# miczi/OpticalFlowHS

Hardware: AMD Instinct MI355X
Metric: Mpixel*iterations/sec (Horn-Schunck: derivative pass + Jacobi u/v sweeps, frames resident in HBM) (higher is better)
Workload: dtype f32; 1 GPU; a stream of 1920x1080 translating-texture pairs resident in HBM, a new pair every step (two seed pairs alternating), lambda 1, 100 Jacobi iterations, ITER|EPS (eps 1e-6) termination; width=1920, height=1080, iters=100, pairs_per_gpu=1, kernel=strip, fuse_steps=20, threads=1024, rows_per_lane_or_groups=5, tiles_per_launch=243, lds_bytes=131328, hipgraph=True, termination=ITER|EPS (eps 1e-6), loop=stream, call=hsflow_pipeline_submit_device, 6 slots on 2 streams, eps_rerun=0

## Files before the change

include/hsflow.h:

```cpp
#ifndef HSFLOW_H_
#define HSFLOW_H_

#include <stddef.h>
#include <stdint.h>

#ifdef __cplusplus
extern "C" {
#endif

#define HSFLOW_VERSION_MAJOR 0
#define HSFLOW_VERSION_MINOR 7

#define HSFLOW_OK 0
#define HSFLOW_E_ARG 1
#define HSFLOW_E_SIZE 2
#define HSFLOW_E_DEVICE 3
#define HSFLOW_E_OOM 4
#define HSFLOW_E_STATE 5
#define HSFLOW_E_NOTERM 6

#define HSFLOW_TERM_ITER 1
#define HSFLOW_TERM_EPS 2

#define HSFLOW_MODE_CV 0
// ... 7 lines not shown
#define HSFLOW_KERNEL_STRIP 3
#define HSFLOW_KERNEL_FOLD 4
#define HSFLOW_KERNEL_PERSIST 5

typedef struct hsflow_ctx hsflow_ctx;

typedef struct hsflow_params {
    uint32_t struct_size;
    int32_t mode;
    float lambda;
    float alpha;
    int32_t term_type;
    int32_t max_iter;
    double epsilon;
    int32_t use_previous;
    int32_t kernel;
    int32_t fuse_steps;
    int32_t tile_w;
    int32_t tile_h;
    int32_t threads;
    int32_t strip_rows;
    int32_t reuse_derivatives;
    int32_t use_graph;
    int32_t profile;
} hsflow_params;

typedef struct hsflow_info {
    uint32_t struct_size;
    int32_t width, height, n_pairs, pitch;
    int32_t iterations_done;
    float last_eps;
    int32_t kernel;
    int32_t fuse_steps, tile_w, tile_h, threads, groups_per_thread;
    int32_t tiles;
    int32_t lds_bytes;
    int32_t jacobi_launches;
    float deriv_ms;
    float jacobi_ms;
    float solve_ms;
    int32_t eps_rerun;
    int32_t deriv_fused;
    int32_t persistent;
} hsflow_info;


void hsflow_default_params(hsflow_params *p);

int hsflow_create(hsflow_ctx **out, int device, int width, int height, int n_pairs, void *stream,
                  int own_stream);
int hsflow_destroy(hsflow_ctx *ctx);
int hsflow_set_row_origin(hsflow_ctx *ctx, int first_row);

int hsflow_set_cu_share(hsflow_ctx *ctx, int compute_units);

int hsflow_set_async_reduce(hsflow_ctx *ctx, int on);

int hsflow_wait_solve(hsflow_ctx *ctx);


int hsflow_set_eps_rows(hsflow_ctx *ctx, int first_row, int rows);
int hsflow_solve_probe(hsflow_ctx *ctx, const hsflow_params *params, float *sweep_eps);
int hsflow_take_verdict(hsflow_ctx *ctx, int *proven);


int hsflow_set_frames_u8(hsflow_ctx *ctx, int pair, const uint8_t *prev, size_t prev_stride,
                         const uint8_t *curr, size_t curr_stride);
int hsflow_set_frames_u8_async(hsflow_ctx *ctx, int pair, const uint8_t *prev, size_t prev_stride,
                               const uint8_t *curr, size_t curr_stride);
int hsflow_set_frames_u8_device(hsflow_ctx *ctx, int pair, const void *d_prev, size_t prev_stride,
                                const void *d_curr, size_t curr_stride);
int hsflow_set_frames_bgr8(hsflow_ctx *ctx, int pair, const uint8_t *prev_bgr, size_t prev_stride,
                           const uint8_t *curr_bgr, size_t curr_stride, int blur3x3);
int hsflow_set_frames_gray8_blur(hsflow_ctx *ctx, int pair, const uint8_t *prev, size_t prev_stride,
                                 const uint8_t *curr, size_t curr_stride);
int hsflow_set_frames_bgr8_async(hsflow_ctx *ctx, int pair, const uint8_t *prev_bgr, size_t prev_stride,
                                 const uint8_t *curr_bgr, size_t curr_stride, int blur3x3);
int hsflow_set_frames_gray8_blur_async(hsflow_ctx *ctx, int pair, const uint8_t *prev, size_t prev_stride,
                                       const uint8_t *curr, size_t curr_stride);
int hsflow_push_frame_u8(hsflow_ctx *ctx, int pair, const uint8_t *next, size_t next_stride);


int hsflow_solve(hsflow_ctx *ctx, const hsflow_params *params);
int hsflow_solve_async(hsflow_ctx *ctx, const hsflow_params *params);
int hsflow_synchronize(hsflow_ctx *ctx);


int hsflow_get_flow(hsflow_ctx *ctx, int pair, float *u, size_t u_stride, float *v, size_t v_stride);
int hsflow_get_flow_async(hsflow_ctx *ctx, int pair, float *u, size_t u_stride, float *v, size_t v_stride);
int hsflow_flow_view_device(hsflow_ctx *ctx, int pair, const float **d_u, const float **d_v, size_t *stride_bytes);
int hsflow_get_flow_device(hsflow_ctx *ctx, int pair, int row0, int nrows, void *d_u,
                           size_t u_stride, void *d_v, size_t v_stride);
int hsflow_set_flow_device(hsflow_ctx *ctx, int pair, int row0, int nrows, const void *d_u,
                           size_t u_stride, const void *d_v, size_t v_stride);
int hsflow_get_derivatives(hsflow_ctx *ctx, int pair, float *dx, float *dy, float *dt,
                           size_t stride);
int hsflow_get_frames_u8(hsflow_ctx *ctx, int pair, uint8_t *prev, size_t prev_stride,
                         uint8_t *curr, size_t curr_stride);


#define HSFLOW_RENDER_CV 0
#define HSFLOW_RENDER_CL 1
typedef struct hsflow_render_params {
    uint32_t struct_size;
    int32_t step;
    float threshold, scale;
    uint8_t dot_rgb[3], line_rgb[3], pad[2];
} hsflow_render_params;
void hsflow_default_render_params(hsflow_render_params *rp, int preset);
int hsflow_render_flow_device(hsflow_ctx *ctx, int pair, const hsflow_render_params *rp, void *d_rgb, size_t stride);
int hsflow_render_flow(hsflow_ctx *ctx, int pair, const hsflow_render_params *rp, uint8_t *rgb, size_t stride);
int hsflow_render_line_pixels(int x0, int y0, int x1, int y1, int width, int height, int32_t *xy, int capacity);


#define HSFLOW_VERIFY_TINY 1e-30f
typedef struct hsflow_plane_diff {
    uint64_t differing, failing, nonfinite;
    int64_t first_failing;
    float max_abs_diff;
    uint32_t max_ulp;
} hsflow_plane_diff;

int hsflow_compare_planes_host(const float *a, size_t a_stride, const float *b, size_t b_stride, int width, int height,
                               hsflow_plane_diff *out);

int hsflow_compare_flow_device(hsflow_ctx *ctx, int pair, const void *d_u, size_t u_stride, const void *d_v, size_t v_stride,
                               hsflow_plane_diff *u, hsflow_plane_diff *v);

typedef struct hsflow_verify_report {
    uint32_t struct_size;
    int32_t ok;
    int32_t pair;
    int32_t iterations_done;
    int32_t iterations_ref;
    int32_t reserved;
    hsflow_plane_diff u, v;
    uint64_t deriv_differing;
    int64_t deriv_first;
} hsflow_verify_report;

int hsflow_verify(hsflow_ctx *ctx, int pair, hsflow_verify_report *report);


int hsflow_get_info(hsflow_ctx *ctx, hsflow_info *info);
int hsflow_get_info_ex(hsflow_ctx *ctx, hsflow_info *info, int measure_last_eps);
const char *hsflow_last_error(hsflow_ctx *ctx);
const char *hsflow_status_string(int status);
int hsflow_version(void);
int hsflow_device_count(int *count);


int hsflow_host_alloc(void **out, size_t bytes);
int hsflow_host_free(void *p);
int hsflow_host_register(void *p, size_t bytes);
int hsflow_host_unregister(void *p);


typedef struct hsflow_pipeline hsflow_pipeline;
int hsflow_pipeline_create(hsflow_pipeline **out, int device, int width, int height, int depth);
int hsflow_pipeline_create_lanes(hsflow_pipeline **out, int device, int width, int height, int depth, int lanes);
int hsflow_pipeline_destroy(hsflow_pipeline *pl);
int hsflow_pipeline_submit(hsflow_pipeline *pl, const uint8_t *prev, size_t prev_stride,
                           const uint8_t *curr, size_t curr_stride, float *u, size_t u_stride,
                           float *v, size_t v_stride, const hsflow_params *params, uint64_t *ticket);
#define HSFLOW_FRAMES_GRAY8 0
#define HSFLOW_FRAMES_GRAY8_BLUR 1
#define HSFLOW_FRAMES_BGR8 2
#define HSFLOW_FRAMES_BGR8_BLUR 3
int hsflow_pipeline_submit_ex(hsflow_pipeline *pl, int format, const uint8_t *prev, size_t prev_stride,
                              const uint8_t *curr, size_t curr_stride, float *u, size_t u_stride,
                              float *v, size_t v_stride, const hsflow_params *params, uint64_t *ticket);
int hsflow_pipeline_submit_device(hsflow_pipeline *pl, const void *d_prev, size_t prev_stride, const void *d_curr,
                                  size_t curr_stride, const hsflow_params *params, uint64_t *ticket);
int hsflow_pipeline_flow_device(hsflow_pipeline *pl, uint64_t ticket, const float **d_u, const float **d_v, size_t *stride_bytes);
int hsflow_pipeline_wait(hsflow_pipeline *pl, uint64_t ticket);
int hsflow_pipeline_render(hsflow_pipeline *pl, uint64_t ticket, const hsflow_render_params *rp, uint8_t *rgb, size_t stride);
int hsflow_pipeline_render_device(hsflow_pipeline *pl, uint64_t ticket, const hsflow_render_params *rp, void *d_rgb, size_t stride);
int hsflow_pipeline_verify(hsflow_pipeline *pl, uint64_t ticket, hsflow_verify_report *report);
int hsflow_pipeline_info(hsflow_pipeline *pl, uint64_t ticket, hsflow_info *info);
int hsflow_pipeline_drain(hsflow_pipeline *pl);
int hsflow_pipeline_depth(hsflow_pipeline *pl);
const char *hsflow_pipeline_last_error(hsflow_pipeline *pl);


typedef struct hsflow_multi hsflow_multi;
int hsflow_multi_create(hsflow_multi **out, const int *devices, int ndev, int width, int height, int depth);
int hsflow_multi_destroy(hsflow_multi *m);
int hsflow_multi_devices(hsflow_multi *m);
int hsflow_multi_submit(hsflow_multi *m, int format, const uint8_t *prev, size_t prev_stride, const uint8_t *curr, size_t curr_stride,
                        float *u, size_t u_stride, float *v, size_t v_stride, const hsflow_params *params, uint64_t *ticket);
int hsflow_multi_wait(hsflow_multi *m, uint64_t ticket);
int hsflow_multi_drain(hsflow_multi *m);
const char *hsflow_multi_last_error(hsflow_multi *m);

typedef struct hsflow_slab hsflow_slab;
int hsflow_slab_create(hsflow_slab **out, const int *devices, int nslab, int width, int height, int halo);
int hsflow_slab_destroy(hsflow_slab *s);
int hsflow_slab_count(hsflow_slab *s);
int hsflow_slab_rows(hsflow_slab *s, int k, int *lo, int *hi);
int hsflow_slab_set_frames_u8(hsflow_slab *s, const uint8_t *prev, size_t prev_stride, const uint8_t *curr, size_t curr_stride);
int hsflow_slab_solve(hsflow_slab *s, const hsflow_params *params);
int hsflow_slab_exchanges(hsflow_slab *s);
int hsflow_slab_iterations_done(hsflow_slab *s);
int hsflow_slab_eps_measured(hsflow_slab *s);
int hsflow_slab_create_overlapped(hsflow_slab **out, const int *devices, int ndev, int width, int height, int halo);
int hsflow_slab_get_flow(hsflow_slab *s, float *u, size_t u_stride, float *v, size_t v_stride);
const char *hsflow_slab_last_error(hsflow_slab *s);

int hsflow_plan_query(int width, int height, int n_pairs, const hsflow_params *params, hsflow_info *info);


int hsflow_calc_optical_flow_hs_8u32f(const uint8_t *prev, const uint8_t *curr, int img_step,
                                      int width, int height, int use_previous, float *velx,
                                      float *vely, int vel_step, float lambda, int term_type,
                                      int max_iter, double epsilon);

void hsflow_release_cached(void);

#ifdef __cplusplus
}
#endif
#endif
```

opticalflowhs_amd/_lib.py:

```python
import ctypes
import os

HERE = os.path.dirname(os.path.abspath(__file__))
LIB_PATH = os.environ.get("HSFLOW_LIB_PATH") or os.path.join(HERE, "libhsflow.so")

OK, E_ARG, E_SIZE, E_DEVICE, E_OOM, E_STATE, E_NOTERM = range(7)
TERM_ITER, TERM_EPS = 1, 2
MODE_CV, MODE_CLASSIC, MODE_CLASSIC_AS_SHIPPED = 0, 1, 2
KERNEL_AUTO, KERNEL_SIMPLE, KERNEL_FUSED, KERNEL_STRIP, KERNEL_FOLD, KERNEL_PERSIST = 0, 1, 2, 3, 4, 5
FRAMES_GRAY8, FRAMES_GRAY8_BLUR, FRAMES_BGR8, FRAMES_BGR8_BLUR = 0, 1, 2, 3
RENDER_CV, RENDER_CL = 0, 1


class HsflowParams(ctypes.Structure):
    _fields_ = [("struct_size", ctypes.c_uint32), ("mode", ctypes.c_int32),
                ("lambda_", ctypes.c_float), ("alpha", ctypes.c_float),
                ("term_type", ctypes.c_int32), ("max_iter", ctypes.c_int32),
                ("epsilon", ctypes.c_double), ("use_previous", ctypes.c_int32),
                ("kernel", ctypes.c_int32), ("fuse_steps", ctypes.c_int32),
                ("tile_w", ctypes.c_int32), ("tile_h", ctypes.c_int32),
                ("threads", ctypes.c_int32), ("strip_rows", ctypes.c_int32),
                ("reuse_derivatives", ctypes.c_int32), ("use_graph", ctypes.c_int32),
                ("profile", ctypes.c_int32)]


class HsflowInfo(ctypes.Structure):
    _fields_ = [("struct_size", ctypes.c_uint32), ("width", ctypes.c_int32),
                ("height", ctypes.c_int32), ("n_pairs", ctypes.c_int32), ("pitch", ctypes.c_int32),
                ("iterations_done", ctypes.c_int32), ("last_eps", ctypes.c_float),
                ("kernel", ctypes.c_int32), ("fuse_steps", ctypes.c_int32),
                ("tile_w", ctypes.c_int32), ("tile_h", ctypes.c_int32), ("threads", ctypes.c_int32),
                ("groups_per_thread", ctypes.c_int32), ("tiles", ctypes.c_int32),
                ("lds_bytes", ctypes.c_int32), ("jacobi_launches", ctypes.c_int32),
                ("deriv_ms", ctypes.c_float), ("jacobi_ms", ctypes.c_float),
                ("solve_ms", ctypes.c_float), ("eps_rerun", ctypes.c_int32),
                ("deriv_fused", ctypes.c_int32), ("persistent", ctypes.c_int32)]


class HsflowRenderParams(ctypes.Structure):
    _fields_ = [("struct_size", ctypes.c_uint32), ("step", ctypes.c_int32),
                ("threshold", ctypes.c_float), ("scale", ctypes.c_float),
                ("dot_rgb", ctypes.c_uint8 * 3), ("line_rgb", ctypes.c_uint8 * 3), ("pad", ctypes.c_uint8 * 2)]


class HsflowPlaneDiff(ctypes.Structure):
    _fields_ = [("differing", ctypes.c_uint64), ("failing", ctypes.c_uint64), ("nonfinite", ctypes.c_uint64),
                ("first_failing", ctypes.c_int64), ("max_abs_diff", ctypes.c_float), ("max_ulp", ctypes.c_uint32)]

    def as_dict(self):
        return {name: getattr(self, name) for name, _ in self._fields_}


class HsflowVerifyReport(ctypes.Structure):
    _fields_ = [("struct_size", ctypes.c_uint32), ("ok", ctypes.c_int32), ("pair", ctypes.c_int32),
                ("iterations_done", ctypes.c_int32), ("iterations_ref", ctypes.c_int32), ("reserved", ctypes.c_int32),
                ("u", HsflowPlaneDiff), ("v", HsflowPlaneDiff),
                ("deriv_differing", ctypes.c_uint64), ("deriv_first", ctypes.c_int64)]


VERIFY_TINY = 1e-30

_vp, _i, _sz = ctypes.c_void_p, ctypes.c_int, ctypes.c_size_t
_pp = ctypes.POINTER(HsflowParams)
_rp = ctypes.POINTER(HsflowRenderParams)
_dp = ctypes.POINTER(HsflowPlaneDiff)
_vr = ctypes.POINTER(HsflowVerifyReport)

PROTOTYPES = {
    "hsflow_default_params": (None, [_pp]),
    "hsflow_create": (_i, [ctypes.POINTER(_vp), _i, _i, _i, _i, _vp, _i]),
    "hsflow_destroy": (_i, [_vp]),
    "hsflow_set_row_origin": (_i, [_vp, _i]),
    "hsflow_set_cu_share": (_i, [_vp, _i]),
    "hsflow_set_async_reduce": (_i, [_vp, _i]),
    "hsflow_set_eps_rows": (_i, [_vp, _i, _i]),
    "hsflow_solve_probe": (_i, [_vp, _pp, ctypes.POINTER(ctypes.c_float)]),
    "hsflow_take_verdict": (_i, [_vp, ctypes.POINTER(_i)]),
    "hsflow_set_frames_u8": (_i, [_vp, _i, _vp, _sz, _vp, _sz]),
    "hsflow_set_frames_u8_async": (_i, [_vp, _i, _vp, _sz, _vp, _sz]),
    "hsflow_set_frames_u8_device": (_i, [_vp, _i, _vp, _sz, _vp, _sz]),
    "hsflow_set_frames_bgr8": (_i, [_vp, _i, _vp, _sz, _vp, _sz, _i]),
    "hsflow_set_frames_gray8_blur": (_i, [_vp, _i, _vp, _sz, _vp, _sz]),
    "hsflow_set_frames_bgr8_async": (_i, [_vp, _i, _vp, _sz, _vp, _sz, _i]),
    "hsflow_set_frames_gray8_blur_async": (_i, [_vp, _i, _vp, _sz, _vp, _sz]),
    "hsflow_push_frame_u8": (_i, [_vp, _i, _vp, _sz]),
    "hsflow_solve": (_i, [_vp, _pp]),
    "hsflow_solve_async": (_i, [_vp, _pp]),
    "hsflow_synchronize": (_i, [_vp]),
    "hsflow_wait_solve": (_i, [_vp]),
    "hsflow_get_flow": (_i, [_vp, _i, _vp, _sz, _vp, _sz]),
    "hsflow_get_flow_async": (_i, [_vp, _i, _vp, _sz, _vp, _sz]),
    "hsflow_flow_view_device": (_i, [_vp, _i, ctypes.POINTER(_vp), ctypes.POINTER(_vp), ctypes.POINTER(_sz)]),
    "hsflow_get_flow_device": (_i, [_vp, _i, _i, _i, _vp, _sz, _vp, _sz]),
    "hsflow_set_flow_device": (_i, [_vp, _i, _i, _i, _vp, _sz, _vp, _sz]),
    "hsflow_get_derivatives": (_i, [_vp, _i, _vp, _vp, _vp, _sz]),
    "hsflow_get_frames_u8": (_i, [_vp, _i, _vp, _sz, _vp, _sz]),
    "hsflow_default_render_params": (None, [_rp, _i]),
    "hsflow_render_flow_device": (_i, [_vp, _i, _rp, _vp, _sz]),
    "hsflow_render_flow": (_i, [_vp, _i, _rp, _vp, _sz]),
    "hsflow_render_line_pixels": (_i, [_i, _i, _i, _i, _i, _i, ctypes.POINTER(ctypes.c_int32), _i]),
    "hsflow_compare_planes_host": (_i, [_vp, _sz, _vp, _sz, _i, _i, _dp]),
    "hsflow_compare_flow_device": (_i, [_vp, _i, _vp, _sz, _vp, _sz, _dp, _dp]),
    "hsflow_verify": (_i, [_vp, _i, _vr]),
    "hsflow_pipeline_verify": (_i, [_vp, ctypes.c_uint64, _vr]),
    "hsflow_get_info": (_i, [_vp, ctypes.POINTER(HsflowInfo)]),
    "hsflow_get_info_ex": (_i, [_vp, ctypes.POINTER(HsflowInfo), _i]),
    "hsflow_last_error": (ctypes.c_char_p, [_vp]),
    "hsflow_status_string": (ctypes.c_char_p, [_i]),
    "hsflow_version": (_i, []),
    "hsflow_device_count": (_i, [ctypes.POINTER(_i)]),
    "hsflow_release_cached": (None, []),
    "hsflow_plan_query": (_i, [_i, _i, _i, _pp, ctypes.POINTER(HsflowInfo)]),
    "hsflow_host_alloc": (_i, [ctypes.POINTER(_vp), _sz]),
    "hsflow_host_free": (_i, [_vp]),
    "hsflow_host_register": (_i, [_vp, _sz]),
    "hsflow_host_unregister": (_i, [_vp]),
    "hsflow_pipeline_create": (_i, [ctypes.POINTER(_vp), _i, _i, _i, _i]),
    "hsflow_pipeline_create_lanes": (_i, [ctypes.POINTER(_vp), _i, _i, _i, _i, _i]),
    "hsflow_pipeline_destroy": (_i, [_vp]),
    "hsflow_pipeline_submit": (_i, [_vp, _vp, _sz, _vp, _sz, _vp, _sz, _vp, _sz, _pp, ctypes.POINTER(ctypes.c_uint64)]),
    "hsflow_pipeline_submit_ex": (_i, [_vp, _i, _vp, _sz, _vp, _sz, _vp, _sz, _vp, _sz, _pp, ctypes.POINTER(ctypes.c_uint64)]),
    "hsflow_pipeline_submit_device": (_i, [_vp, _vp, _sz, _vp, _sz, _pp, ctypes.POINTER(ctypes.c_uint64)]),
    "hsflow_pipeline_flow_device": (_i, [_vp, ctypes.c_uint64, ctypes.POINTER(_vp), ctypes.POINTER(_vp), ctypes.POINTER(_sz)]),
    "hsflow_pipeline_wait": (_i, [_vp, ctypes.c_uint64]),
    "hsflow_pipeline_render": (_i, [_vp, ctypes.c_uint64, _rp, _vp, _sz]),
    "hsflow_pipeline_render_device": (_i, [_vp, ctypes.c_uint64, _rp, _vp, _sz]),
    "hsflow_pipeline_info": (_i, [_vp, ctypes.c_uint64, ctypes.POINTER(HsflowInfo)]),
    "hsflow_pipeline_drain": (_i, [_vp]),
    "hsflow_pipeline_depth": (_i, [_vp]),
    "hsflow_pipeline_last_error": (ctypes.c_char_p, [_vp]),
    "hsflow_multi_create": (_i, [ctypes.POINTER(_vp), ctypes.POINTER(_i), _i, _i, _i, _i]),
    "hsflow_multi_destroy": (_i, [_vp]),
    "hsflow_multi_devices": (_i, [_vp]),
    "hsflow_multi_submit": (_i, [_vp, _i, _vp, _sz, _vp, _sz, _vp, _sz, _vp, _sz, _pp, ctypes.POINTER(ctypes.c_uint64)]),
    "hsflow_multi_wait": (_i, [_vp, ctypes.c_uint64]),
    "hsflow_multi_drain": (_i, [_vp]),
    "hsflow_multi_last_error": (ctypes.c_char_p, [_vp]),
    "hsflow_slab_create": (_i, [ctypes.POINTER(_vp), ctypes.POINTER(_i), _i, _i, _i, _i]),
    "hsflow_slab_destroy": (_i, [_vp]),
    "hsflow_slab_count": (_i, [_vp]),
    "hsflow_slab_rows": (_i, [_vp, _i, ctypes.POINTER(_i), ctypes.POINTER(_i)]),
    "hsflow_slab_set_frames_u8": (_i, [_vp, _vp, _sz, _vp, _sz]),
    "hsflow_slab_solve": (_i, [_vp, _pp]),
    "hsflow_slab_exchanges": (_i, [_vp]),
    "hsflow_slab_iterations_done": (_i, [_vp]),
    "hsflow_slab_eps_measured": (_i, [_vp]),
    "hsflow_slab_create_overlapped": (_i, [ctypes.POINTER(_vp), ctypes.POINTER(_i), _i, _i, _i, _i]),
    "hsflow_slab_get_flow": (_i, [_vp, _vp, _sz, _vp, _sz]),
    "hsflow_slab_last_error": (ctypes.c_char_p, [_vp]),
    "hsflow_calc_optical_flow_hs_8u32f": (_i, [_vp, _vp, _i, _i, _i, _i, _vp, _vp, _i,
                                               ctypes.c_float, _i, _i, ctypes.c_double]),
}

_lib = None


def load():
    global _lib
    if _lib is not None:
        return _lib
    try:
        import torch
    except ImportError:
        pass
    if not os.path.exists(LIB_PATH):
        raise ImportError(
            "opticalflowhs_amd: %s is missing -- build it with `python opticalflowhs_amd/build.py` "
            "(hipcc, gfx950). There is no CPU fallback." % LIB_PATH)
    try:
        lib = ctypes.CDLL(LIB_PATH)
    except OSError as e:
        raise ImportError("opticalflowhs_amd: cannot load %s: %s" % (LIB_PATH, e))
    for name, (res, args) in PROTOTYPES.items():
        try:
            fn = getattr(lib, name)
        except AttributeError:
            raise ImportError("opticalflowhs_amd: %s does not export %s" % (LIB_PATH, name))
        fn.restype = res
        fn.argtypes = args
    _lib = lib
    return lib


class HsflowError(RuntimeError):
    def __init__(self, status, message):
        RuntimeError.__init__(self, "hsflow status %d: %s" % (status, message))
        self.status = status
```

opticalflowhs_amd/csrc/hs_context.hip.h:

```cpp
#pragma once

namespace {

constexpr int kMaxFuse = 32;
constexpr int kLdsLimit = 160 * 1024;
constexpr int kNumCU = 256;

thread_local std::string g_create_error;

struct FusedPlan {
    hsk::FusedGeom g;
    int NT, K, lds_bytes, tiles;
};

struct StripPlan {
    hsk::StripGeom g;
    int R, lds_bytes, tiles;
    int fold;
};

struct JPlan {
    int kind = 0;
    int T = 0;
    FusedPlan f{};
// ... 29 lines not shown
};

struct SolveSetup {
    float coeff;
    int kernel;
    bool multi;
    bool use_iter, use_eps;
    long long budget;
    int T;
    JPlan plan;
    bool persist;
    hsflow_params eff;
};

struct PlanKey {
    hsflow_params p;
    int async, exact;
};
struct PlanEntry {
    PlanKey key;
    SolveSetup S;
    hsflow_info info;
};

}

struct hsflow_ctx {
    int device = 0;
    int W = 0, H = 0, N = 0, P = 0;
    int org = 0;
    long long plane = 0;
    hipStream_t stream = nullptr;
    bool own_stream = false;
    uint8_t *dA = nullptr, *dB = nullptr;
    uint32_t *dCoef = nullptr;
    float *dE[3] = {nullptr, nullptr, nullptr};
    bool dE_valid = false;
    int coef_mode = -1;
    float *dU[2] = {nullptr, nullptr}, *dV[2] = {nullptr, nullptr};
    unsigned long long *dStamps = nullptr;
    unsigned *dEps = nullptr;
    unsigned *epsPtr = nullptr;
    float epsThr = 0.f;
    unsigned *hEps = nullptr;
    unsigned *hEpsDev = nullptr;
    size_t hEpsCap = 0;
    int epsStride = 1;
    unsigned *dEpsTiles = nullptr;
    size_t epsTilesCap = 0;
    float *dUb = nullptr, *dVb = nullptr;
    float *dUp = nullptr, *dVp = nullptr;
    unsigned *dFlags = nullptr;
    unsigned *hErr = nullptr, *hErrDev = nullptr;
    int persist_tiles = 0;
    bool persist_off = false;
    bool persist_unchecked = false;
    bool counted = false;
    int eps_row0 = 0, eps_rows = 0;
    std::vector<float> sweep_eps;
    unsigned *dSeq = nullptr, *hMark = nullptr, *hMarkDev = nullptr;
    float *dZero = nullptr;
    unsigned mark_issued = 0;
    bool last_marked = false;
    bool flow_after_mark = false;
    bool async_reduce = false;
    int cu_share = 0;
    int num_cu = 0;
    int max_grid_z = 65535;
    void *dScratch = nullptr;
    unsigned *dPrio = nullptr;
    bool prio_dirty = false;
    uint8_t *dRgb = nullptr;
    hipEvent_t evRender = nullptr;
    hsflow_params vparams;
    int vstate = 0;
    int v_org = 0, v_eps_row0 = 0, v_eps_rows = 0;
    hsflow_ctx *shadow = nullptr;
    bool borrowed = false;
    unsigned long long *dCmp = nullptr, *hCmp = nullptr;
    int cmp_cap = 0;
    hipEvent_t evVerify = nullptr;
    size_t scratch_bytes = 0;
    int cur = 0;
    bool frames_set = false;
    bool coef_valid = false;
    hsflow_info info;
    std::string err;
    struct Pending {
        bool active = false;
        hsflow_params params;
        int iters = 0, launches = 0, cur0 = 0;
        EpsLayout words;
        bool reduced = false;
        unsigned mark = 0;
        bool marked_by_reduce = false;
    } pend;
    struct LastLaunch {
        bool valid = false;
        JPlan plan;
        int zero_in = 0;
        float coeff = 0.f, eps_thr = 0.f;
        bool from_third = false;
    } lastl;
    bool force_exact = false;
    bool configuring = false;
    std::map<GraphKey, GraphEntry> graphs;
    std::vector<PlanEntry> plan_cache;
    std::vector<hipEvent_t> events;
};

namespace {

std::atomic<int> g_live_ctx[64];
constexpr int kMaxPersistTiles = 4096;

hsflow_ctx *g_oneshot = nullptr;
std::mutex g_oneshot_mutex;

int fail(hsflow_ctx *c, int code, const std::string &msg)
{
    if (c) c->err = msg; else g_create_error = msg;
    return code;
}

#define HS_HIP(c, call)                                                                           \
    do {                                                                                          \
        hipError_t e_ = (call);                                                                   \
        if (e_ != hipSuccess)                                                                     \
            return fail((c), e_ == hipErrorOutOfMemory ? HSFLOW_E_OOM : HSFLOW_E_DEVICE,          \
                        std::string(#call) + ": " + hipGetErrorString(e_));                       \
    } while (0)

int round_up(int v, int m) { return (v + m - 1) / m * m; }

}
```

opticalflowhs_amd/csrc/hs_kernels_strip.hip.h:

```cpp
#pragma once
#include <type_traits>

#ifndef HS_SCALED
#define HS_SCALED 1
#endif
#ifndef HS_UNROLL2_FOLD
#define HS_UNROLL2_FOLD 1
#endif
#ifndef HS_PEEL_LAST_STRIP
#define HS_PEEL_LAST_STRIP 1
#endif
#ifndef HS_PEEL_LAST_FOLD
#define HS_PEEL_LAST_FOLD 1
#endif
#ifndef HS_CORE_PRIO
#define HS_CORE_PRIO 1
#endif
#ifndef HS_SWEEP_STAMPS
#define HS_SWEEP_STAMPS 0
#endif
#ifndef HS_DIAG
#define HS_DIAG 0
#endif

// ... 47 lines not shown
}
__device__ __forceinline__ f4 load_f4_sc1(__amdgpu_buffer_rsrc_t rs, unsigned row_bytes, unsigned lane_bytes)
{
    return __builtin_bit_cast(f4, __builtin_amdgcn_raw_buffer_load_b128(rs, (int)lane_bytes, (int)row_bytes, 16));
}
__device__ __forceinline__ unsigned load_u32_sc1(const unsigned *p)
{
    return __hip_atomic_load(p, __ATOMIC_RELAXED, __HIP_MEMORY_SCOPE_AGENT);
}

__device__ __forceinline__ int hs_lane_now()
{
    unsigned m = ~0u;
    asm volatile("" : "+s"(m));
    return (int)__builtin_amdgcn_mbcnt_hi(m, __builtin_amdgcn_mbcnt_lo(m, 0u));
}

__device__ __forceinline__ f2 f2_fma(f2 a, f2 b, f2 c) { return __builtin_elementwise_fma(a, b, c); }
__device__ __forceinline__ f2 f2_swap(f2 a) { return __builtin_shufflevector(a, a, 1, 0); }
#if HS_SCALED
#define HS_DIFF(o, n) f2_fma((o), f2{4.0f, 4.0f}, -(n))
#define HS_DIFF1(o, n) fmaf(4.0f, (o), -(n))
#else
#define HS_DIFF(o, n) ((o) - (n))
#define HS_DIFF1(o, n) ((o) - (n))
#endif

struct RowCoef { f2 alP, alQ, beP, beQ, gaP, gaQ; };

struct Cross { f2 uP, uQ, vP, vQ; };

__device__ __forceinline__ f2 pk_add_swapped(f2 a, f2 b)
{
    f2 r;
    asm("v_pk_add_f32 %0, %1, %2 op_sel:[0,1] op_sel_hi:[1,0]" : "=v"(r) : "v"(a), "v"(b));
    return r;
}

template <int E>
__device__ __forceinline__ void cross_rows(Cross &s, const f2 cuP, const f2 cuQ, const f2 cvP, const f2 cvQ,
                                           const f2 duP, const f2 duQ, const f2 dvP, const f2 dvQ)
{
    if (E == 0) {
        s.uP = duP + cuQ; s.uQ = duQ + cuP;
        s.vP = dvP + cvQ; s.vQ = dvQ + cvP;
    } else {
        s.uQ = pk_add_swapped(duQ, cuQ);
        s.uP.x = duP.x + wave_from_prev_lane(cuP.y); s.uP.y = duP.y + wave_from_next_lane(cuP.x);
        s.vQ = pk_add_swapped(dvQ, cvQ);
        s.vP.x = dvP.x + wave_from_prev_lane(cvP.y); s.vP.y = dvP.y + wave_from_next_lane(cvP.x);
    }
}

template <int E>
__device__ __forceinline__ void strip_row_update(f2 &uP, f2 &uQ, f2 &vP, f2 &vQ, const Cross &sc, const Cross &sp, RowCoef &c)
{
    f2 tP, tQ, sP, sQ;
    if (E == 0) {
        tQ = pk_add_swapped(sc.uQ, sp.uQ);
        tP.x = sc.uP.x + wave_from_prev_lane(sp.uP.y); tP.y = sc.uP.y + wave_from_next_lane(sp.uP.x);
        sQ = pk_add_swapped(sc.vQ, sp.vQ);
        sP.x = sc.vP.x + wave_from_prev_lane(sp.vP.y); sP.y = sc.vP.y + wave_from_next_lane(sp.vP.x);
    } else {
        tP = sc.uP + sp.uQ; tQ = sc.uQ + sp.uP;
        sP = sc.vP + sp.vQ; sQ = sc.vQ + sp.vP;
    }
#if HS_SCALED
    const f2 ubP = tP, ubQ = tQ, vbP = sP, vbQ = sQ;
#else
    const f2 ubP = tP * 0.25f, ubQ = tQ * 0.25f, vbP = sP * 0.25f, vbQ = sQ * 0.25f;
#endif
    const f2 qP = f2_fma(c.alP, ubP, f2_fma(c.beP, vbP, c.gaP));
    const f2 qQ = f2_fma(c.alQ, ubQ, f2_fma(c.beQ, vbQ, c.gaQ));
    uP = f2_fma(-c.alP, qP, ubP);
    vP = f2_fma(-c.beP, qP, vbP);
    uQ = f2_fma(-c.alQ, qQ, ubQ);
    vQ = f2_fma(-c.beQ, qQ, vbQ);
#if HS_SCALED
    c.gaP *= 4.0f;
    c.gaQ *= 4.0f;
#endif
}

template <int R>
__device__ __forceinline__ void strip_derive(const uint8_t *__restrict__ fA, const uint8_t *__restrict__ fB,
                                             const StripGeom &g, long long base, int x0, int y0, int dir, bool xin,
                                             uint4 (&lc)[R])
{
    const int mode = xin ? 0 : ((x0 < 0 || (g.W & 3) == 0) ? 1 : 2);
    int xg = x0, xb[4] = {0, 0, 0, 0};
    unsigned flipx = 0;
    if (mode == 1) {
        xg = x0 < 0 ? -x0 - 4 : 2 * g.W - x0 - 4;
        if (xg < 0 || xg + 4 > g.W) xg = 0;
        flipx = 0xFu;
    } else if (mode == 2) {
#pragma unroll
        for (int k = 0; k < 4; k++) {
            xb[k] = mirror_index(x0 + k, g.W);
            if (x0 + k >= g.W) flipx |= 1u << k;
        }
    }
    uint32_t wa[R + 2], wbv[R];
#pragma unroll
    for (int j = 0; j < R + 2; j++)
        wa[j] = *(const uint32_t *)(fA + base + (long long)mirror_index(y0 + dir * (j - 1), g.H) * g.P + (mode == 2 ? 0 : xg));
#pragma unroll
    for (int r = 0; r < R; r++)
        wbv[r] = *(const uint32_t *)(fB + base + (long long)mirror_index(y0 + dir * r, g.H) * g.P + (mode == 2 ? 0 : xg));
    if (mode == 1) {
#pragma unroll
        for (int j = 0; j < R + 2; j++) wa[j] = __builtin_bswap32(wa[j]);
#pragma unroll
        for (int r = 0; r < R; r++) wbv[r] = __builtin_bswap32(wbv[r]);
    }
    if (__builtin_amdgcn_ballot_w64(mode == 2) != 0) {
        if (mode == 2) {
            auto bytes = [&](const uint8_t *row) -> uint32_t {
                return (uint32_t)row[xb[0]] | ((uint32_t)row[xb[1]] << 8) | ((uint32_t)row[xb[2]] << 16) | ((uint32_t)row[xb[3]] << 24);
            };
#pragma unroll
            for (int j = 0; j < R + 2; j++) wa[j] = bytes(fA + base + (long long)mirror_index(y0 + dir * (j - 1), g.H) * g.P);
#pragma unroll
            for (int r = 0; r < R; r++) wbv[r] = bytes(fB + base + (long long)mirror_index(y0 + dir * r, g.H) * g.P);
        }
    }
    int a[R + 2][6];
#pragma unroll
    for (int j = 0; j < R + 2; j++) {
        const uint32_t wd = wa[j];
        a[j][0] = (int)((uint32_t)__builtin_amdgcn_update_dpp(0, (int)wd, 0x138, 0xF, 0xF, true) >> 24);
        a[j][5] = (int)((uint32_t)__builtin_amdgcn_update_dpp(0, (int)wd, 0x130, 0xF, 0xF, true) & 0xFFu);
#pragma unroll
        for (int k = 0; k < 4; k++) a[j][k + 1] = (int)((wd >> (8 * k)) & 0xFFu);
    }
#pragma unroll
    for (int r = 0; r < R; r++) {
        const int y = y0 + dir * r;
        const uint32_t wb = wbv[r];
        const bool yflip = (y < 0 || y >= g.H) != (dir < 0);
        uint32_t o[4];
#pragma unroll
        for (int k = 0; k < 4; k++) {
            int ix8 = (a[r][k + 2] + 2 * a[r + 1][k + 2] + a[r + 2][k + 2]) - (a[r][k] + 2 * a[r + 1][k] + a[r + 2][k]);
            int iy8 = (a[r + 2][k] + 2 * a[r + 2][k + 1] + a[r + 2][k + 2]) - (a[r][k] + 2 * a[r][k + 1] + a[r][k + 2]);
            if ((flipx >> k) & 1u) ix8 = -ix8;
            if (yflip) iy8 = -iy8;
            o[k] = pack_deriv(ix8, iy8, (int)((wb >> (8 * k)) & 0xFFu) - a[r + 1][k + 1]);
        }
        lc[r] = make_uint4(o[0], o[1], o[2], o[3]);
    }
}

template <int R, int NTMAX, int EPS, int E0, bool DERIV, bool PERSIST = false>
__device__ __forceinline__ void strip_body(const uint32_t *__restrict__ coef,
                                                        const float *__restrict__ u_in,
                                                        const float *__restrict__ v_in,
                                                        float *__restrict__ u_out,
                                                        float *__restrict__ v_out, const StripGeom g,
                                                        const float ilambda,
                                                        unsigned *__restrict__ eps_out, const int eps_stride,
                                                        unsigned long long *__restrict__ stamps,
                                                        const float eps_thr, const uint8_t *__restrict__ fA,
                                                        const uint8_t *__restrict__ fB, uint32_t *__restrict__ coef_w,
                                                        const PersistArgs pa = PersistArgs())
{
    static_assert(!PERSIST || EPS == 0 || EPS == 2, "the persistent form runs plain or witness phases");
    extern __shared__ __attribute__((aligned(16))) float4 ex[];
    unsigned long long st0 = 0, sr0 = 0, st1 = 0, st2 = 0;
    if (stamps) { st0 = __builtin_amdgcn_s_memtime(); sr0 = __builtin_amdgcn_s_memrealtime(); }
    const int lane = threadIdx.x & 63;
    const int w = __builtin_amdgcn_readfirstlane(threadIdx.x >> 6);
    const int NW = g.NW;
    float *eps_lds = (float *)(ex + (size_t)2 * NW * 4 * 64);
    const int tpp = g.tiles_x * g.tiles_y;
    const int tile = xcd_contiguous_tile(blockIdx.x, gridDim.x);
    const int pair = tile / tpp;
    const int t2 = tile - pair * tpp;
    const int by = t2 / g.tiles_x, bx = t2 - by * g.tiles_x;
    const int x0 = bx * g.CW - g.HX + 4 * lane;
    const int y0 = by * g.CH - g.T + w * R;
    const long long base = (long long)pair * g.plane;
    const bool xin = (x0 >= 0) && (x0 + 3 < g.W);
    const bool rev = (R & 1) != 0 && ((y0 + g.org) & 1) != 0;
    auto img_row = [&](int r) { return rev ? R - 1 - r : r; };

    f2 uP[R], uQ[R], vP[R], vQ[R];
    RowCoef cf[R];
    float4 lu[R], lv[R];
    uint4 lc[R];
    const int rx0 = bx * g.CW - g.HX;
    const bool xedge = !(rx0 >= 0 && rx0 + 256 <= g.W);
    int xg = x0;
    bool xrev = false, slow = false;
    if (xedge && !xin) {
        if (x0 < 0 && -x0 <= g.W) { xg = -x0 - 4; xrev = true; }
        else if (x0 >= g.W && (g.W & 3) == 0 && 2 * g.W - x0 - 4 >= 0) { xg = 2 * g.W - x0 - 4; xrev = true; }
        else { xg = 0; slow = true; }
    }
#pragma unroll
    for (int r = 0; r < R; r++) {
        const long long off = base + (long long)mirror_index(y0 + img_row(r), g.H) * g.P + xg;
        const long long off_uv = g.zero_in ? (long long)xg : off;
        lc[r] = make_uint4(0u, 0u, 0u, 0u);
        if constexpr (!DERIV) {
            lu[r] = *(const float4 *)(u_in + off_uv);
            lv[r] = *(const float4 *)(v_in + off_uv);
            lc[r] = *(const uint4 *)(coef + off);
        } else {
            lu[r] = lv[r] = make_float4(0.f, 0.f, 0.f, 0.f);
        }
    }
    if constexpr (DERIV) {
        if (!g.zero_in) {
#pragma unroll
            for (int r = 0; r < R; r++) {
                const long long off = base + (long long)mirror_index(y0 + img_row(r), g.H) * g.P + xg;
                lu[r] = *(const float4 *)(u_in + off);
                lv[r] = *(const float4 *)(v_in + off);
            }
        }
    }
    auto unpack_row = [&](const int r) __attribute__((always_inline)) {
        const float4 lu_ = lu[r], lv_ = lv[r];
        const uint4 cw = lc[r];
        constexpr int iPx = 0, iPy = 3, iQx = 1, iQy = 2;
        const float lu4[4] = {lu_.x, lu_.y, lu_.z, lu_.w}, lv4[4] = {lv_.x, lv_.y, lv_.z, lv_.w};
        uP[r] = f2{lu4[iPx], lu4[iPy]}; uQ[r] = f2{lu4[iQx], lu4[iQy]};
        vP[r] = f2{lv4[iPx], lv4[iPy]}; vQ[r] = f2{lv4[iQx], lv4[iQy]};
        float al[4], be[4], ga[4];
        const uint32_t cc[4] = {cw.x, cw.y, cw.z, cw.w};
#pragma unroll
        for (int p = 0; p < 4; p++) sweep_coefs(cc[p], ilambda, al[p], be[p], ga[p]);
        cf[r].alP = f2{al[iPx], al[iPy]}; cf[r].alQ = f2{al[iQx], al[iQy]};
        cf[r].beP = f2{be[iPx], be[iPy]}; cf[r].beQ = f2{be[iQx], be[iQy]};
        cf[r].gaP = f2{ga[iPx], ga[iPy]} * (HS_SCALED ? 4.0f : 1.0f); cf[r].gaQ = f2{ga[iQx], ga[iQy]} * (HS_SCALED ? 4.0f : 1.0f);
    };
    if constexpr (!DERIV) {
#pragma unroll
        for (int r = 0; r < R; r++) unpack_row(r);
    }
    if (xedge) {
#pragma unroll
        for (int r = 0; r < R; r++) {
            if constexpr (DERIV) {
                if (xrev) {
                    lu[r] = make_float4(lu[r].w, lu[r].z, lu[r].y, lu[r].x);
                    lv[r] = make_float4(lv[r].w, lv[r].z, lv[r].y, lv[r].x);
                }
            } else {
                uP[r] = xrev ? f2_swap(uP[r]) : uP[r]; uQ[r] = xrev ? f2_swap(uQ[r]) : uQ[r];
                vP[r] = xrev ? f2_swap(vP[r]) : vP[r]; vQ[r] = xrev ? f2_swap(vQ[r]) : vQ[r];
                cf[r].alP = xrev ? f2_swap(cf[r].alP) : cf[r].alP; cf[r].alQ = xrev ? f2_swap(cf[r].alQ) : cf[r].alQ;
                cf[r].beP = xrev ? f2_swap(cf[r].beP) : cf[r].beP; cf[r].beQ = xrev ? f2_swap(cf[r].beQ) : cf[r].beQ;
                cf[r].gaP = xrev ? f2_swap(cf[r].gaP) : cf[r].gaP; cf[r].gaQ = xrev ? f2_swap(cf[r].gaQ) : cf[r].gaQ;
            }
        }
        if (__builtin_amdgcn_ballot_w64(slow) != 0) {
            if (slow) {
                const int xa = mirror_index(x0, g.W), xb = mirror_index(x0 + 1, g.W),
                          xc = mirror_index(x0 + 2, g.W), xd = mirror_index(x0 + 3, g.W);
#pragma unroll
                for (int r = 0; r < R; r++) {
                    const long long row = base + (long long)mirror_index(y0 + img_row(r), g.H) * g.P;
                    {
                        const float *uv = u_in + (g.zero_in ? 0 : row), *vv = v_in + (g.zero_in ? 0 : row);
                        lu[r] = make_float4(uv[xa], uv[xb], uv[xc], uv[xd]);
                        lv[r] = make_float4(vv[xa], vv[xb], vv[xc], vv[xd]);
                    }
                    if constexpr (!DERIV) {
                        const uint32_t *cv = coef + row;
                        lc[r] = make_uint4(cv[xa], cv[xb], cv[xc], cv[xd]);
                        unpack_row(r);
                    }
                }
            }
        }
    }
    if constexpr (DERIV) {
        strip_derive<R>(fA, fB, g, base, x0, rev ? y0 + R - 1 : y0, rev ? -1 : 1, xin, lc);
#pragma unroll
        for (int r = 0; r < R; r++) unpack_row(r);
    }
    unsigned rowcore = 0;
    int rdist[R];
#pragma unroll
    for (int r = 0; r < R; r++) {
        const int j = w * R + img_row(r), y = y0 + img_row(r);
        if (j >= g.T && j < g.T + g.CH && y >= 0 && y < g.H) rowcore |= 1u << r;
        rdist[r] = j < g.T ? g.T - j : (j >= g.T + g.CH ? j - (g.T + g.CH - 1) : 0);
    }
    const bool lanecore = (x0 >= 0) && (x0 < g.W) && (4 * lane >= g.HX) && (4 * lane < g.HX + g.CW);
    const int pr = g.W - 1 - x0;
    const int lane_kept = lane;
    constexpr bool LANE_HW = EPS != 0 || PERSIST;
#define lane (LANE_HW ? hs_lane_now() : lane_kept)
    unsigned epscore = 0;
    if (EPS != 0) {
#pragma unroll
        for (int r = 0; r < R; r++) {
            const int y = y0 + img_row(r);
            if (((rowcore >> r) & 1u) && y >= g.ey0 && y < g.ey1) epscore |= 1u << r;
        }
    }
    if (DERIV && lanecore) {
#pragma unroll
        for (int r = 0; r < R; r++)
            if ((rowcore >> r) & 1u) *(uint4 *)(coef_w + base + (long long)(y0 + img_row(r)) * g.P + x0) = lc[r];
    }

#define HS_ACT(r) (rdist[r] <= last)
#define HS_ROW(r, PE, SC, SP)                                                                      \
    do {                                                                                           \
        if (HS_ACT(r)) {                                                                           \
            f2 ouP, ouQ, ovP, ovQ;                                                                 \
            if (EM == 1) { ouP = uP[r]; ouQ = uQ[r]; ovP = vP[r]; ovQ = vQ[r]; }                   \
            if (HS_DIAG & 8) uP[r] += SC.uP + SP.uP;                                               \
            else strip_row_update<PE>(uP[r], uQ[r], vP[r], vQ[r], SC, SP, cf[r]);                  \
            if (EM == 1) {                                                                         \
                if ((epscore >> (r)) & 1u) {  \
                    const f2 dUP = HS_DIFF(ouP, uP[r]), dUQ = HS_DIFF(ouQ, uQ[r]), dVP = HS_DIFF(ovP, vP[r]), dVQ = HS_DIFF(ovQ, vQ[r]); \
                    if (!xedge) {  \
                        e = fmaxf(fmaxf(e, fabsf(dUP.x)), fabsf(dUP.y));                           \
                        e = fmaxf(fmaxf(e, fabsf(dUQ.x)), fabsf(dUQ.y));                           \
                        e = fmaxf(fmaxf(e, fabsf(dVP.x)), fabsf(dVP.y));                           \
                        e = fmaxf(fmaxf(e, fabsf(dVQ.x)), fabsf(dVQ.y));                           \
                    } else {                                                                       \
                         \
                        e = fmaxf(e, fmaxf(fabsf(dUP.x), fabsf(dVP.x)));                           \
                        if (pr >= 1) e = fmaxf(e, fmaxf(fabsf(dUQ.x), fabsf(dVQ.x)));              \
                        if (pr >= 2) e = fmaxf(e, fmaxf(fabsf(dUQ.y), fabsf(dVQ.y)));              \
                        if (pr >= 3) e = fmaxf(e, fmaxf(fabsf(dUP.y), fabsf(dVP.y)));              \
                    }                                                                              \
                }                                                                                  \
            }                                                                                      \
        }                                                                                          \
    } while (0)
#define HS_CROSS(S, PE, A, B)                                                                      \
    do {                                                                                           \
        if (HS_ACT(A) || HS_ACT(B)) {                                                              \
            if (HS_DIAG & 8) S.uP = uP[A] + uP[B];                                                 \
            else cross_rows<PE>(S, uP[A], uQ[A], vP[A], vQ[A], uP[B], uQ[B], vP[B], vQ[B]);        \
        }                                                                                          \
    } while (0)
#define HS_PUBLISH(buf)                                                                            \
    do {                                                                                           \
        float4 *exw = ex + ((size_t)((buf) * NW + w) * 4) * 64 + HS_LANE;                          \
        exw[0] = make_float4(uP[0].x, uP[0].y, uQ[0].x, uQ[0].y);                                  \
        exw[64] = make_float4(vP[0].x, vP[0].y, vQ[0].x, vQ[0].y);                                 \
        exw[128] = make_float4(uP[R - 1].x, uP[R - 1].y, uQ[R - 1].x, uQ[R - 1].y);                \
        exw[192] = make_float4(vP[R - 1].x, vP[R - 1].y, vQ[R - 1].x, vQ[R - 1].y);                \
    } while (0)

    if (stamps) st1 = __builtin_amdgcn_s_memtime();
    const bool nrev = (R & 1) != 0 && !rev;
    const int wa = w > 0 ? w - 1 : w, sa = w > 0 ? (nrev ? 0 : 2) : 0;
    const int wb = w < NW - 1 ? w + 1 : w, sb = w < NW - 1 ? (nrev ? 2 : 0) : 2;
    const int wu = rev ? wb : wa, su = rev ? sb : sa;
    const int wd = rev ? wa : wb, sd = rev ? sa : sb;
    int seen_n = 0;
    const unsigned long long wit_mask = (epscore & 1u) ? __builtin_amdgcn_ballot_w64(lanecore) : 0ull;
    const int core_here = min(g.CH, g.H - by * g.CH);
    const int wit_lo = (g.T + R - 1) / R, wit_n = (g.T + core_here) / R - wit_lo;
// ... 213 lines not shown
                if (nx >= 0 && nx < g.tiles_x && ny >= 0 && ny < g.tiles_y) nb = pair * tpp + ny * g.tiles_x + nx;
            } else if (lane == 8) nb = (int)gridDim.x;
            const unsigned long long t0 = __builtin_amdgcn_s_memrealtime();
            int dead = 0;
            for (;;) {
                unsigned v = target;
                if (nb >= 0) v = load_u32_sc1(pa.flags + nb);
                const bool aborted = lane == 8 && v != 0u;
                const bool behind = lane < 8 && (int)(v - target) < 0;
                if (__builtin_amdgcn_ballot_w64(aborted) != 0) { dead = 1; break; }
                if (__builtin_amdgcn_ballot_w64(behind) == 0) break;
                if (__builtin_amdgcn_s_memrealtime() - t0 > (unsigned long long)pa.wait_ticks) {
                    dead = 1;
                    if (lane == 0) {
                        __hip_atomic_store(pa.flags + gridDim.x, 1u, __ATOMIC_RELAXED, __HIP_MEMORY_SCOPE_AGENT);
                        __hip_atomic_store(pa.err, 1u, __ATOMIC_RELAXED, __HIP_MEMORY_SCOPE_SYSTEM);
                    }
                    break;
                }
                __builtin_amdgcn_s_sleep(4);
            }
            if (lane == 0) *dead_lds = dead;
        }
        __syncthreads();
        if (__builtin_amdgcn_readfirstlane(*dead_lds)) return;
        if (stamps) { const unsigned long long t = __builtin_amdgcn_s_memtime(); pt_wait += t - pt0; pt0 = t; }
        {
            f4 tu[R], tv[R];
#pragma unroll
            for (int r = 0; r < R; r++) {
                const unsigned row = 4u * (unsigned)(base + (long long)mirror_index(y0 + img_row(r), g.H) * g.P);
                tu[r] = f4{uP[r].x, uQ[r].x, uQ[r].y, uP[r].y};
                tv[r] = f4{vP[r].x, vQ[r].x, vQ[r].y, vP[r].y};
                if (!((rowcore >> r) & 1u) || !lanecore) {
                    tu[r] = load_f4_sc1(pu, row, 4u * (unsigned)xgx);
                    tv[r] = load_f4_sc1(pv, row, 4u * (unsigned)xgx);
                }
            }
#pragma unroll
            for (int r = 0; r < R; r++) {
                if (xrevx) {
                    tu[r] = f4{tu[r].w, tu[r].z, tu[r].y, tu[r].x};
                    tv[r] = f4{tv[r].w, tv[r].z, tv[r].y, tv[r].x};
                }
                uP[r] = f2{tu[r].x, tu[r].w}; uQ[r] = f2{tu[r].y, tu[r].z};
                vP[r] = f2{tv[r].x, tv[r].w}; vQ[r] = f2{tv[r].y, tv[r].z};
            }
        }
        ph++;
    }
    }
#undef HS_ROW
#undef HS_ACT
#undef HS_CROSS
#undef HS_PUBLISH
#undef HS_LANE
#undef lane
    if (stamps && threadIdx.x == 0) {
        __builtin_amdgcn_s_waitcnt(0);
        unsigned long long *o = stamps + (size_t)blockIdx.x * 8;
        o[0] = st0; o[1] = st1; o[2] = st2; o[3] = __builtin_amdgcn_s_memtime();
        o[4] = sr0; o[5] = __builtin_amdgcn_s_memrealtime();
        o[6] = (unsigned long long)__builtin_amdgcn_s_getreg(((4 - 1) << 11) | (0 << 6) | 20);
        o[7] = (unsigned long long)tile;
        if (PERSIST && gridDim.x <= 8192) {
            unsigned long long *q = stamps + (size_t)gridDim.x * 8 + (size_t)blockIdx.x * 32;
            q[0] = pt_sweep; q[1] = pt_pub; q[2] = pt_wait; q[3] = pt_load; q[4] = pt_first - st1; q[5] = o[3] - st2;
        }
    }
}

template <int R, int NTMAX, int EPS, int E0>
__global__ __launch_bounds__(NTMAX) void k_jacobi_strip(const uint32_t *__restrict__ coef,
                                                        const float *__restrict__ u_in,
                                                        const float *__restrict__ v_in,
                                                        float *__restrict__ u_out,
                                                        float *__restrict__ v_out, const StripGeom g,
                                                        const float ilambda,
                                                        unsigned *__restrict__ eps_out, const int eps_stride,
                                                        unsigned long long *__restrict__ stamps,
                                                        const float eps_thr)
{
    strip_body<R, NTMAX, EPS, E0, false>(coef, u_in, v_in, u_out, v_out, g, ilambda, eps_out, eps_stride, stamps, eps_thr,
                                     nullptr, nullptr, nullptr);
}

template <int R, int NTMAX, int EPS, int E0>
__global__ __launch_bounds__(NTMAX) void k_jacobi_strip_deriv(const uint8_t *__restrict__ fA,
                                                              const uint8_t *__restrict__ fB,
                                                              uint32_t *__restrict__ coef_w,
                                                              const float *__restrict__ u_in,
                                                              const float *__restrict__ v_in,
                                                              float *__restrict__ u_out,
                                                              float *__restrict__ v_out, const StripGeom g,
                                                              const float ilambda,
                                                              unsigned *__restrict__ eps_out, const int eps_stride,
                                                              unsigned long long *__restrict__ stamps,
                                                              const float eps_thr)
{
    strip_body<R, NTMAX, EPS, E0, true>(nullptr, u_in, v_in, u_out, v_out, g, ilambda, eps_out, eps_stride, stamps, eps_thr,
                                    fA, fB, coef_w);
}

template <int R, int NTMAX, int EPS, int E0, bool DERIV>
__global__ __launch_bounds__(NTMAX) void k_jacobi_strip_persist(const uint8_t *__restrict__ fA,
                                                                const uint8_t *__restrict__ fB,
                                                                uint32_t *coef_rw,
                                                                const float *__restrict__ u_in,
                                                                const float *__restrict__ v_in, const StripGeom g,
                                                                const float ilambda,
                                                                unsigned *__restrict__ eps_out, const int eps_stride,
                                                                unsigned long long *__restrict__ stamps,
                                                                const float eps_thr, const PersistArgs pa)
{
    strip_body<R, NTMAX, EPS, E0, DERIV, true>(coef_rw, u_in, v_in, nullptr, nullptr, g, ilambda, eps_out, eps_stride, stamps, eps_thr,
                                               fA, fB, coef_rw, pa);
}

__device__ __forceinline__ float lane_xor32(float x, bool lower)
{
    const unsigned b = __float_as_uint(x);
    const auto r = __builtin_amdgcn_permlane32_swap(b, b, false, false);
    return __uint_as_float(lower ? r[0] : r[1]);
}

template <int R, int NTMAX, int EPS, int E0, bool DERIV>
__device__ __forceinline__ void fold_body(const uint32_t *__restrict__ coef,
                                                       const float *__restrict__ u_in,
                                                       const float *__restrict__ v_in,
                                                       float *__restrict__ u_out,
                                                       float *__restrict__ v_out, const StripGeom g,
                                                       const float ilambda,
                                                       unsigned *__restrict__ eps_out, const int eps_stride,
                                                       unsigned long long *__restrict__ stamps,
                                                       const float eps_thr, const uint8_t *__restrict__ fA,
                                                       const uint8_t *__restrict__ fB, uint32_t *__restrict__ coef_w)
{
    extern __shared__ __attribute__((aligned(16))) float4 ex[];
    unsigned long long st0 = 0, sr0 = 0, st1 = 0, st2 = 0;
    if (stamps) { st0 = __builtin_amdgcn_s_memtime(); sr0 = __builtin_amdgcn_s_memrealtime(); }
    const int lane = threadIdx.x & 63, hl = lane & 31;
    const bool lower = lane >= 32;
    const int w = __builtin_amdgcn_readfirstlane(threadIdx.x >> 6);
    const int NW = g.NW;
    float *eps_lds = (float *)(ex + (size_t)2 * NW * 2 * 2 * 32);
    const int tpp = g.tiles_x * g.tiles_y;
    const int tile = xcd_contiguous_tile(blockIdx.x, gridDim.x);
    const int pair = tile / tpp;
    const int t2 = tile - pair * tpp;
    const int by = t2 / g.tiles_x, bx = t2 - by * g.tiles_x;
    const int rx0 = bx * g.CW - g.HX;
    const int x0 = rx0 + 4 * hl;
    const int yb = by * g.CH - g.T + w * 2 * R;
    const long long base = (long long)pair * g.plane;
    const bool xin = (x0 >= 0) && (x0 + 3 < g.W);

    f2 uP[R], uQ[R], vP[R], vQ[R];
    RowCoef cf[R];
    float4 lu[R], lv[R];
    uint4 lc[R];
    const bool side = !(rx0 >= 0 && rx0 + 128 <= g.W);
    int xg = x0;
    bool rev = false, slow = false;
    if (side && !xin) {
        if (x0 < 0 && -x0 <= g.W) { xg = -x0 - 4; rev = true; }
        else if (x0 >= g.W && (g.W & 3) == 0 && 2 * g.W - x0 - 4 >= 0) { xg = 2 * g.W - x0 - 4; rev = true; }
        else { xg = 0; slow = true; }
    }
#pragma unroll
    for (int r = 0; r < R; r++) {
        const int y = yb + (lower ? 2 * R - 1 - r : r);
        const long long off = base + (long long)mirror_index(y, g.H) * g.P + xg;
        const long long off_uv = g.zero_in ? (long long)xg : off;
        lc[r] = make_uint4(0u, 0u, 0u, 0u);
        if constexpr (!DERIV) {
            lu[r] = *(const float4 *)(u_in + off_uv);
            lv[r] = *(const float4 *)(v_in + off_uv);
            lc[r] = *(const uint4 *)(coef + off);
        } else {
            lu[r] = lv[r] = make_float4(0.f, 0.f, 0.f, 0.f);
        }
    }
    if constexpr (DERIV) {
        if (!g.zero_in) {
#pragma unroll
            for (int r = 0; r < R; r++) {
                const int y = yb + (lower ? 2 * R - 1 - r : r);
                const long long off = base + (long long)mirror_index(y, g.H) * g.P + xg;
                lu[r] = *(const float4 *)(u_in + off);
                lv[r] = *(const float4 *)(v_in + off);
            }
        }
    }
    auto unpack_row = [&](const int r) __attribute__((always_inline)) {
        constexpr int iPx = 0, iPy = 3, iQx = 1, iQy = 2;
        const float lu4[4] = {lu[r].x, lu[r].y, lu[r].z, lu[r].w}, lv4[4] = {lv[r].x, lv[r].y, lv[r].z, lv[r].w};
        uP[r] = f2{lu4[iPx], lu4[iPy]}; uQ[r] = f2{lu4[iQx], lu4[iQy]};
        vP[r] = f2{lv4[iPx], lv4[iPy]}; vQ[r] = f2{lv4[iQx], lv4[iQy]};
        float al[4], be[4], ga[4];
// ... 264 lines not shown
```

opticalflowhs_amd/csrc/hs_plan_launch.hip.h:

```cpp
#pragma once

namespace {
int eps_row0(const hsflow_ctx *c) { return c->eps_rows > 0 ? c->eps_row0 : 0; }
int eps_row1(const hsflow_ctx *c) { return c->eps_rows > 0 ? c->eps_row0 + c->eps_rows : c->H; }
bool eps_windowed(const hsflow_ctx *c) { return c->eps_rows > 0 && (c->eps_row0 > 0 || c->eps_rows < c->H); }

int plan_cus(const hsflow_ctx *c) { return c->cu_share > 0 ? c->cu_share : kNumCU; }
bool plan_shared(const hsflow_ctx *c) { return c->cu_share > 0 && c->cu_share < kNumCU; }

bool grid_fits(long long tiles, int threads) { return tiles * threads <= 0xFFFFFFFFLL; }

bool make_plan(const hsflow_ctx *c, int T, int tw, int th, int nt, FusedPlan &best)
{
    const int W = c->W, H = c->H;
    const int HX = round_up(T, 4);
    double best_cost = 1e300;
    bool found = false;
    const int nts[3] = {1024, 512, 256};
    for (int nti = 0; nti < 3; nti++) {
        const int NT = nts[nti];
        if (nt && nt != NT) continue;
        const int Kmax = NT == 1024 ? 3 : 4;
        const int wg_per_cu = 1;
        const int cw_lo = tw ? tw : 4, cw_hi = tw ? tw : std::min(round_up(W, 4), 1024);
// ... 234 lines not shown
    const double valu = std::max(wps, 1.0) * R * instr_per_row * cpi * (1.0 - 0.45 * halo_frac);
    const double exchange = 300.0 + (fold ? 12.0 : 20.0) * NW * conc;
    const double sweep = valu + exchange;
    double load = 2050.0 + 0.4 * 256.0 * R * NW * conc;
    if (conc > 1) load *= 0.4;
    const double r = (double)tiles / (double)slots;
    const double rounds = plan_shared(c) ? std::max(1.0, r) : conc == 1 ? std::ceil(r) : std::max(1.0, r + 0.7);
    return 6000.0 + 6e-4 * 8.0 * image_pixels + rounds * (load + T * sweep);
}

bool make_strip_plan(const hsflow_ctx *c, int T, int rows, int threads, int fold, StripPlan &best, double *cost_out = nullptr)
{
    const int W = c->W, H = c->H;
    const int HX = round_up(T, 4);
    const int CW = (fold ? 128 : 256) - 2 * HX;
    if (CW < 4) return false;
    double best_cost = 1e300;
    bool found = false;
    for (int R = 1; R <= 8; R++) {
        if (rows && rows != R) continue;
        for (int NW = 1; NW <= strip_max_waves(R, fold); NW++) {
            if (threads && threads != NW * 64) continue;
            const int CH = NW * R * (fold ? 2 : 1) - 2 * T;
            if (CH < 1) continue;
            const int lds = NW * (fold ? 4096 : 8192) + (fold ? 128 : 256);
            if (lds > kLdsLimit) continue;
            const int tx = (W + CW - 1) / CW, ty = (H + CH - 1) / CH;
            const long long tiles = (long long)tx * ty * c->N;
            if (!grid_fits(tiles, NW * 64)) continue;
            const double cost = strip_launch_cost(c, T, R, NW, tiles, fold, (double)W * H * c->N);
            if (cost < best_cost - 1e-9) {
                best_cost = cost;
                found = true;
                best.R = R;
                best.fold = fold;
                best.lds_bytes = lds;
                best.tiles = (int)tiles;
                hsk::StripGeom &g = best.g;
                g.W = W; g.H = H; g.P = c->P; g.plane = c->plane;
                g.T = T; g.HX = HX; g.CW = CW; g.CH = CH; g.NW = NW;
                g.tiles_x = tx; g.tiles_y = ty; g.zero_in = 0; g.org = c->org;
                g.ey0 = eps_row0(c); g.ey1 = eps_row1(c);
            }
        }
    }
    if (cost_out) *cost_out = best_cost;
    return found;
}

int pick_strip_T(const hsflow_ctx *c, int iters, const hsflow_params &p, int fold, double *total_out = nullptr)
{
    double best = 1e300;
    int bestT = 1;
    for (int T = 1; T <= std::min(iters, 24); T++) {
        StripPlan sp;
        double cfull = 0, ctail = 0;
        if (!make_strip_plan(c, T, p.strip_rows, p.threads, fold, sp, &cfull)) continue;
        const int rem = iters % T;
        if (rem && !make_strip_plan(c, rem, p.strip_rows, p.threads, fold, sp, &ctail)) continue;
        const double total = (iters / T) * cfull + (rem ? ctail : 0.0);
        if (total < best) { best = total; bestT = T; }
    }
    if (total_out) *total_out = best;
    return bestT;
}

int strip_phase(const StripPlan &p) { return (p.fold || (p.R & 1) == 0) ? ((p.g.T + p.g.org) & 1) : 0; }

template <int R, int NTMAX, int EPS, bool FOLD, bool DERIV, int E0>
constexpr auto strip_kernel()
{
    if constexpr (FOLD && DERIV) return hsk::k_jacobi_fold_deriv<R, NTMAX, EPS, E0>;
    else if constexpr (FOLD) return hsk::k_jacobi_fold<R, NTMAX, EPS, E0>;
    else if constexpr (DERIV) return hsk::k_jacobi_strip_deriv<R, NTMAX, EPS, E0>;
    else return hsk::k_jacobi_strip<R, NTMAX, EPS, E0>;
}

template <int R, int NTMAX, EpsMode EPS, bool FOLD, bool DERIV, int E0>
hipError_t launch_strip_k(const hsflow_ctx *c, const StripPlan &p, const float *ui, const float *vi, float *uo, float *vo, float coeff)
{
    constexpr auto kern = strip_kernel<R, NTMAX, (int)EPS, FOLD, DERIV, E0>();
    if (p.g.zero_in) ui = vi = c->dZero;
    unsigned long long *stamps = p.tiles <= 65536 ? c->dStamps : nullptr;
    if constexpr (DERIV)
        return launch_lds<kern>(c, p.tiles, p.g.NW * 64, p.lds_bytes, c->dA, c->dB, c->dCoef, ui, vi, uo, vo, p.g, coeff, c->epsPtr,
                                c->epsStride, stamps, c->epsThr);
    else
        return launch_lds<kern>(c, p.tiles, p.g.NW * 64, p.lds_bytes, c->dCoef, ui, vi, uo, vo, p.g, coeff, c->epsPtr, c->epsStride,
                                stamps, c->epsThr);
}

template <int R, int NTMAX, EpsMode EPS, bool FOLD, bool DERIV>
hipError_t launch_strip_t(const hsflow_ctx *c, const StripPlan &p, const float *ui, const float *vi, float *uo, float *vo, float coeff)
{
    if constexpr (FOLD || (R & 1) == 0) {
        if (strip_phase(p)) return launch_strip_k<R, NTMAX, EPS, FOLD, DERIV, 1>(c, p, ui, vi, uo, vo, coeff);
    }
    return launch_strip_k<R, NTMAX, EPS, FOLD, DERIV, 0>(c, p, ui, vi, uo, vo, coeff);
}

constexpr int strip_ntmax(int R, bool fold, bool narrow)
{
    return R <= 4 ? 1024 : R == 5 ? (fold || narrow ? 768 : 1024) : R == 6 ? (fold ? 512 : 768) : 512;
}

template <int R, EpsMode EPS, bool FOLD, bool DERIV>
hipError_t launch_strip_r(const hsflow_ctx *c, const StripPlan &p, const float *ui, const float *vi, float *uo, float *vo, float coeff)
{
    constexpr int NT = strip_ntmax(R, FOLD, false), NT_NARROW = strip_ntmax(R, FOLD, EPS != EpsMode::None);
    if constexpr (NT_NARROW != NT) {
        if (p.g.NW <= 12) return launch_strip_t<R, NT_NARROW, EPS, FOLD, DERIV>(c, p, ui, vi, uo, vo, coeff);
    }
    return launch_strip_t<R, NT, EPS, FOLD, DERIV>(c, p, ui, vi, uo, vo, coeff);
}

template <EpsMode EPS, bool FOLD, bool DERIV>
hipError_t launch_strip_e(const hsflow_ctx *c, const StripPlan &p, const float *ui, const float *vi, float *uo, float *vo, float coeff)
{
#ifdef HS_DIAG_MIN
    if constexpr (!FOLD && !DERIV && EPS == EpsMode::None) {
        if (p.R == 4) return launch_strip_r<4, EPS, FOLD, DERIV>(c, p, ui, vi, uo, vo, coeff);
        if (p.R == 5) return launch_strip_r<5, EPS, FOLD, DERIV>(c, p, ui, vi, uo, vo, coeff);
        if (p.R == 6) return launch_strip_r<6, EPS, FOLD, DERIV>(c, p, ui, vi, uo, vo, coeff);
    }
#else
    switch (p.R) {
    case 1: return launch_strip_r<1, EPS, FOLD, DERIV>(c, p, ui, vi, uo, vo, coeff);
    case 2: return launch_strip_r<2, EPS, FOLD, DERIV>(c, p, ui, vi, uo, vo, coeff);
    case 3: return launch_strip_r<3, EPS, FOLD, DERIV>(c, p, ui, vi, uo, vo, coeff);
    case 4: return launch_strip_r<4, EPS, FOLD, DERIV>(c, p, ui, vi, uo, vo, coeff);
    case 5: return launch_strip_r<5, EPS, FOLD, DERIV>(c, p, ui, vi, uo, vo, coeff);
    case 6: return launch_strip_r<6, EPS, FOLD, DERIV>(c, p, ui, vi, uo, vo, coeff);
    }
    if constexpr (!DERIV) {
        if (p.R == 7) return launch_strip_r<7, EPS, FOLD, DERIV>(c, p, ui, vi, uo, vo, coeff);
        if (p.R == 8) return launch_strip_r<8, EPS, FOLD, DERIV>(c, p, ui, vi, uo, vo, coeff);
    }
#endif
    return hipErrorInvalidConfiguration;
}

template <EpsMode EPS>
hipError_t launch_strip_m(const hsflow_ctx *c, const StripPlan &p, bool deriv, const float *ui, const float *vi, float *uo, float *vo,
                          float coeff)
{
    if constexpr (EPS != EpsMode::EverySweep) {
        if (deriv) return p.fold ? launch_strip_e<EPS, true, true>(c, p, ui, vi, uo, vo, coeff)
                                 : launch_strip_e<EPS, false, true>(c, p, ui, vi, uo, vo, coeff);
    }
    if (deriv) return hipErrorInvalidConfiguration;
    return p.fold ? launch_strip_e<EPS, true, false>(c, p, ui, vi, uo, vo, coeff)
                  : launch_strip_e<EPS, false, false>(c, p, ui, vi, uo, vo, coeff);
}

constexpr unsigned kPersistWaitTicks = 5000000u;

const char *persist_obstacle(const hsflow_ctx *c, const StripPlan &sp, int iters, const hsflow_params &p, bool async, bool use_eps)
{
    static const bool off = getenv("HSFLOW_NO_PERSIST") != nullptr;
    const hsk::StripGeom &g = sp.g;
    if (off) return "HSFLOW_NO_PERSIST is set";
    if (c->persist_off) return "a persistent launch timed out on this context earlier";
    if (sp.fold) return "the folded kernel has no persistent form";
    if (sp.R != 5 || g.NW * 64 > 1024) return "the persistent form is compiled for 5 rows per lane";
    if (iters <= g.T) return "a single phase";
    if ((g.W & 3) != 0 || g.W < 256 || g.H < g.NW * sp.R) return "the frame must be at least one region large and its width a multiple of 4";
    if (g.CH < g.T || g.CW < g.HX) return "the halo reaches past the neighbouring tiles";
// ... 170 lines not shown
```

opticalflowhs_amd/csrc/hs_runtime.hip.h:

```cpp
#pragma once

namespace {
constexpr size_t kMaxGraphs = 32;
void drop_graphs(hsflow_ctx *c)
{
    if (c->graphs.empty()) return;
    hipStreamSynchronize(c->stream);
    for (auto &kv : c->graphs) {
        if (kv.second.exec) hipGraphExecDestroy(kv.second.exec);
        if (kv.second.graph) hipGraphDestroy(kv.second.graph);
    }
    c->graphs.clear();
}

void trim_graph_cache(hsflow_ctx *c)
{
    if (c->graphs.size() >= kMaxGraphs) drop_graphs(c);
}

int check_ctx(hsflow_ctx *c, int pair)
{
    if (!c) return fail(nullptr, HSFLOW_E_ARG, "null context");
    if (pair < 0 || pair >= c->N) return fail(c, HSFLOW_E_ARG, "pair index out of range");
    if (hipSetDevice(c->device) != hipSuccess) return fail(c, HSFLOW_E_DEVICE, "hipSetDevice failed");
    (void)hipGetLastError();
    return HSFLOW_OK;
}

struct Profiler {
    hsflow_ctx *c;
    bool on;
    std::vector<std::pair<int, size_t>> marks;
    size_t used = 0;
    hipEvent_t ev(size_t i)
    {
        while (c->events.size() <= i) {
            hipEvent_t e;
            if (hipEventCreate(&e) != hipSuccess) return nullptr;
            c->events.push_back(e);
        }
        return c->events[i];
    }
    void begin(int kind)
    {
        if (!on) return;
        marks.push_back({kind, used});
        hipEventRecord(ev(used), c->stream);
        used++;
    }
    void end()
    {
        if (!on) return;
        hipEventRecord(ev(used), c->stream);
        used++;
    }
    void collect()
    {
        if (!on || marks.empty()) return;
        hipStreamSynchronize(c->stream);
        float d = 0, j = 0, t = 0;
        for (auto &m : marks) {
            float ms = 0;
            hipEventElapsedTime(&ms, c->events[m.second], c->events[m.second + 1]);
            (m.first == 0 ? d : j) += ms;
        }
        hipEventElapsedTime(&t, c->events[marks.front().second], c->events[used - 1]);
        c->info.deriv_ms = d;
        c->info.jacobi_ms = j;
        c->info.solve_ms = t;
    }
};

int persist_reserve(hsflow_ctx *c)
{
    const size_t px = (size_t)c->plane * c->N;
    if (!c->dUp) HS_HIP(c, hipMalloc((void **)&c->dUp, px * sizeof(float)));
    if (!c->dVp) HS_HIP(c, hipMalloc((void **)&c->dVp, px * sizeof(float)));
    if (!c->dFlags) {
        HS_HIP(c, hipMalloc((void **)&c->dFlags, (size_t)(kMaxPersistTiles + 1) * sizeof(unsigned)));
        c->persist_tiles = 0;
    }
    if (!c->hErr) {
        HS_HIP(c, hipHostMalloc((void **)&c->hErr, 64, hipHostMallocMapped | hipHostMallocCoherent));
        HS_HIP(c, hipHostGetDevicePointer((void **)&c->hErrDev, c->hErr, 0));
        *c->hErr = 0u;
    }
    return HSFLOW_OK;
}

int persist_prepare_flags(hsflow_ctx *c, int tiles)
{
    if (c->persist_tiles == tiles) return HSFLOW_OK;
    HS_HIP(c, hipMemsetAsync(c->dFlags, 0, (size_t)(kMaxPersistTiles + 1) * sizeof(unsigned), c->stream));
    c->persist_tiles = tiles;
    return HSFLOW_OK;
}

void persist_failed(hsflow_ctx *c)
{
    if (c->hErr) *c->hErr = 0u;
    c->persist_tiles = 0;
    c->persist_off = true;
    c->persist_unchecked = false;
    c->coef_valid = false;
    c->plan_cache.clear();
}

bool persist_error(const hsflow_ctx *c) { return c->hErr && *(volatile unsigned *)c->hErr != 0u; }

bool persist_gave_up(hsflow_ctx *c)
{
    const bool gave_up = c->persist_unchecked && persist_error(c);
    c->persist_unchecked = false;
    if (gave_up) persist_failed(c);
    return gave_up;
}

int enqueue_persist(hsflow_ctx *c, const StripPlan &sp0, int iters, EpsMode eps, bool deriv, int zero_in, float coeff)
{
    StripPlan sp = sp0;
    sp.g.zero_in = zero_in;
    hsk::PersistArgs pa;
    const int T = sp.g.T;
    pa.n_phase = (iters + T - 1) / T;
    pa.T_last = iters - (pa.n_phase - 1) * T;
    pa.flags = c->dFlags;
    pa.err = c->hErrDev;
    static const char *ticks_env = getenv("HSFLOW_PERSIST_WAIT_TICKS");
    pa.wait_ticks = ticks_env ? (unsigned)strtoul(ticks_env, nullptr, 10) : kPersistWaitTicks;
    const int a = c->cur, b = a ^ 1;
    const int lastb = (pa.n_phase - 1) & 1;
    pa.ub[lastb] = c->dU[b]; pa.vb[lastb] = c->dV[b];
    pa.ub[lastb ^ 1] = c->dUp; pa.vb[lastb ^ 1] = c->dVp;
    HS_HIP(c, launch_persist(c, sp, pa, eps, deriv, c->dU[a], c->dV[a], coeff));
    c->cur = b;
    return HSFLOW_OK;
}

int configure_persist(hsflow_ctx *c, const StripPlan &sp, EpsMode eps, bool deriv, float coeff)
{
    c->configuring = true;
    const hipError_t e = launch_persist(c, sp, hsk::PersistArgs{}, eps, deriv, nullptr, nullptr, coeff);
    c->configuring = false;
    HS_HIP(c, e);
    return HSFLOW_OK;
}

int enqueue_fixed(hsflow_ctx *c, const hsflow_params &p, float coeff, int iters, int kernel, int T,
                  const JPlan *plan, const JPlan *tail_plan, Profiler &prof, bool do_deriv, bool zero_flow, bool persist = false)
{
    int zero_in = zero_flow ? 1 : 0;
    if (zero_flow) c->cur = 0;
    bool fuse = do_deriv && !p.profile && kernel != HSFLOW_KERNEL_SIMPLE &&
                strip_deriv_fusable(c, iters >= T ? *plan : *tail_plan);
    if (do_deriv && !fuse) {
        prof.begin(0);
        HS_HIP(c, launch_deriv(c));
        prof.end();
    }
    int left = iters, launches = 0;
    if (persist) {
        prof.begin(1);
        const int st = enqueue_persist(c, plan->s, iters, EpsMode::None, fuse, zero_in, coeff);
        prof.end();
        if (st) return st;
        left = 0;
        launches = 1;
    }
    while (left > 0) {
        const int a = c->cur, b = a ^ 1;
        if (kernel == HSFLOW_KERNEL_SIMPLE) {
            prof.begin(1);
            HS_HIP(c, launch_simple(c, false, c->dU[a], c->dV[a], c->dU[b], c->dV[b], coeff, zero_in));
            prof.end();
            left -= 1;
        } else {
            const JPlan *pl = (left >= T) ? plan : tail_plan;
            prof.begin(1);
            HS_HIP(c, launch_j(c, *pl, EpsMode::None, c->dU[a], c->dV[a], c->dU[b], c->dV[b], coeff, zero_in, fuse));
            prof.end();
            fuse = false;
            left -= pl->T;
        }
        c->cur = b;
        zero_in = 0;
        launches++;
    }
    c->info.jacobi_launches = launches;
    return HSFLOW_OK;
}

int eps_reserve(hsflow_ctx *c, int sweeps, int stride)
{
    const size_t need = (size_t)sweeps * stride;
    if (c->epsTilesCap < need) {
        drop_graphs(c);
        hipFree(c->dEpsTiles);
        c->dEpsTiles = nullptr; c->epsTilesCap = 0;
        HS_HIP(c, hipMalloc((void **)&c->dEpsTiles, need * sizeof(unsigned)));
        c->epsTilesCap = need;
    }
    if (c->hEpsCap < (size_t)sweeps) {
        drop_graphs(c);
        HS_HIP(c, hipStreamSynchronize(c->stream));
        if (c->hEps) hipHostFree(c->hEps);
        c->hEps = c->hEpsDev = nullptr; c->hEpsCap = 0;
        const size_t cap = std::max<size_t>(256, (size_t)sweeps * 2);
        HS_HIP(c, hipHostMalloc((void **)&c->hEps, cap * sizeof(unsigned), hipHostMallocMapped | hipHostMallocCoherent));
        HS_HIP(c, hipHostGetDevicePointer((void **)&c->hEpsDev, c->hEps, 0));
        c->hEpsCap = cap;
    }
    c->epsStride = stride;
    return HSFLOW_OK;
}

int eps_clear(hsflow_ctx *c, int sweeps, int stride)
{
    HS_HIP(c, hipMemsetAsync(c->dEpsTiles, 0, (size_t)sweeps * stride * sizeof(unsigned), c->stream));
    return HSFLOW_OK;
}

int eps_prepare(hsflow_ctx *c, int sweeps, int stride)
{
    const int st = eps_reserve(c, sweeps, stride);
    return st ? st : eps_clear(c, sweeps, stride);
}

int eps_collect_enqueue(hsflow_ctx *c, const EpsLayout &w, bool mark = false)
{
    c->epsPtr = c->dEps;
    c->epsStride = 1;
    if (c->configuring) return HSFLOW_OK;
    hipLaunchKernelGGL(hsk::k_eps_reduce, dim3(w.slots), dim3(256), 0, c->stream, c->dEpsTiles, w.stride, c->hEpsDev, w.n_first,
                       w.cnt_first, w.cnt_last, mark ? c->dSeq : nullptr, mark ? c->hMarkDev : nullptr);
    HS_HIP(c, hipGetLastError());
    return HSFLOW_OK;
}

int eps_collect(hsflow_ctx *c, int sweeps, std::vector<unsigned> &host)
{
    int st = eps_collect_enqueue(c, EpsLayout{sweeps, c->epsStride, 0, 0, c->epsStride});
    if (st) return st;
    HS_HIP(c, hipStreamSynchronize(c->stream));
    host.assign(c->hEps, c->hEps + sweeps);
    return HSFLOW_OK;
}

bool witness_proven(const unsigned *w, int slots, double epsilon, float *last, bool last_is_exact)
{
    float e = 0.f;
    for (int i = 0; i < slots; i++) {
        std::memcpy(&e, &w[i], sizeof(float));
        if (!((double)e >= epsilon) && !(last_is_exact && i == slots - 1)) return false;
    }
    *last = e;
    return true;
}

int plan_eps_stride(int kernel, const JPlan &pl) { return (kernel == HSFLOW_KERNEL_STRIP || kernel == HSFLOW_KERNEL_FOLD) ? pl.s.tiles : 1; }

constexpr int kStampTiles = 65536;
void dump_stamps(hsflow_ctx *c, int tiles)
{
    const char *path = getenv("HSFLOW_DEBUG_STAMPS");
    if (!path || !c->dStamps) return;
    tiles = std::min(tiles, kStampTiles);
    std::vector<unsigned long long> h((size_t)tiles * 8);
    if (hipMemcpy(h.data(), c->dStamps, h.size() * 8, hipMemcpyDeviceToHost) != hipSuccess) return;
    FILE *f = fopen(path, "a");
// ... 39 lines not shown
```

opticalflowhs_amd/csrc/hs_solve.hip.h:

```cpp
#pragma once

namespace {
int solve_impl(hsflow_ctx *c, const hsflow_params *pp, bool async);

int check_persist(hsflow_ctx *c)
{
    if (!persist_gave_up(c)) return HSFLOW_OK;
    return fail(c, HSFLOW_E_DEVICE, "a persistent launch of an asynchronous solve timed out (another grid on the device?): its flow is invalid; "
                                    "this context now launches per fuse_steps iterations, solve again");
}

int wait_marker(hsflow_ctx *c, unsigned target)
{
    if (!c->hMark) { HS_HIP(c, hipStreamSynchronize(c->stream)); return HSFLOW_OK; }
    const auto t0 = std::chrono::steady_clock::now();
    unsigned spins = 0;
    while ((int)(__atomic_load_n(c->hMark, __ATOMIC_ACQUIRE) - target) < 0) {
        if ((++spins & 1023u) == 0 && std::chrono::steady_clock::now() - t0 > std::chrono::seconds(2)) {
            HS_HIP(c, hipStreamSynchronize(c->stream));
            break;
        }
    }
    return HSFLOW_OK;
}
// ... 199 lines not shown
    const bool do_unpack = need_planes && (do_deriv || !c->dE_valid);
    auto enqueue = [&](int *n) -> int {
        if (do_deriv) {
            prof.begin(0);
            HS_HIP(c, for_pair_batches(c, [&](long long o, int pairs) {
                hipLaunchKernelGGL(hsk::k_deriv_classic_packed, grid(pairs), block, 0, c->stream, c->dA + o, c->dB + o, c->dCoef + o,
                                   c->W, c->H, c->P, c->plane);
            }));
            prof.end();
        }
        if (do_unpack) {
            HS_HIP(c, for_pair_batches(c, [&](long long o, int pairs) {
                hipLaunchKernelGGL(hsk::k_unpack_classic_deriv, grid(pairs), block, 0, c->stream, c->dCoef + o, c->dE[0] + o, c->dE[1] + o,
                                   c->dE[2] + o, c->W, c->H, c->P, c->plane);
            }));
        }
        int zero = zero0 ? 1 : 0;
        if (zero) c->cur = 0;
        int done = 0, launches = 0;
        while (done < p.max_iter) {
            const int chunk = std::min(T, p.max_iter - done);
            const int a = c->cur, b = a ^ 1;
            prof.begin(1);
            hipError_t e;
            if (kernel == HSFLOW_KERNEL_STRIP) {
                ClassicStripPlan cp = chunk == T ? splan : stail;
                cp.g.zero_in = zero;
                e = launch_classic_strip(c, cp, write_v, c->dU[a], c->dV[a], c->dU[b], c->dV[b], a2);
            } else if (kernel == HSFLOW_KERNEL_FUSED) {
                FusedPlan cp = chunk == T ? fplan : ftail;
                cp.g.zero_in = zero;
                e = launch_classic_fused(c, cp, write_v, c->dU[a], c->dV[a], c->dU[b], c->dV[b], a2);
            } else {
                auto kern = zero ? (write_v ? hsk::k_jacobi_classic<true, true> : hsk::k_jacobi_classic<true, false>)
                                 : (write_v ? hsk::k_jacobi_classic<false, true> : hsk::k_jacobi_classic<false, false>);
                e = for_pair_batches(c, [&](long long o, int pairs) {
                    hipLaunchKernelGGL(kern, grid(pairs), block, 0, c->stream, c->dE[0] + o, c->dE[1] + o, c->dE[2] + o, c->dU[a] + o,
                                       c->dV[a] + o, c->dU[b] + o, c->dV[b] + o, c->W, c->H, c->P, c->plane, a2);
                });
            }
            prof.end();
            HS_HIP(c, e);
            c->cur = b;
            zero = 0;
            done += chunk;
            launches++;
        }
        *n = launches;
        return HSFLOW_OK;
    };
    hsflow_info &i = c->info;
    int launches = 0;
    if (p.use_graph) {
        GraphKey key{p.mode, kernel, p.max_iter, T, i.tile_w, i.tile_h, i.threads, i.groups_per_thread, zero0 ? 0 : c->cur,
                     p.use_previous * 2 + (do_deriv ? 1 : 0) + (do_unpack ? 4 : 0), p.alpha};
        if ((st = run_captured(c, key, enqueue, &launches))) return st;
    } else if ((st = enqueue(&launches))) return st;
    c->coef_valid = true;
    c->coef_mode = HSFLOW_MODE_CLASSIC;
    c->dE_valid = do_unpack || (c->dE_valid && !do_deriv);
    i.jacobi_launches = launches;
    i.iterations_done = p.max_iter; i.last_eps = 0.f; i.deriv_ms = i.jacobi_ms = i.solve_ms = 0.f;
    if (!async) {
        HS_HIP(c, hipStreamSynchronize(c->stream));
        prof.collect();
    }
    return HSFLOW_OK;
}

int solve_fixed(hsflow_ctx *c, const hsflow_params &p, const SolveSetup &S, Profiler &prof, bool async)
{
    const int iters = (int)S.budget, T = S.T;
    int st = HSFLOW_OK;
    JPlan tail;
    const int rem = (S.multi && !S.persist) ? iters % T : 0;
    if (rem && !make_jplan(c, S.kernel, rem, p, tail))
        return fail(c, HSFLOW_E_SIZE, "no feasible launch plan for the tail launch");
    const bool zero = !p.use_previous;
    const bool do_deriv = !(p.reuse_derivatives && c->coef_valid && c->coef_mode == HSFLOW_MODE_CV);
    c->info.deriv_fused = do_deriv && !p.profile && S.multi && strip_deriv_fusable(c, iters >= T ? S.plan : tail);
    if (S.persist) {
        if ((st = persist_reserve(c)) || (st = persist_prepare_flags(c, S.plan.s.tiles))) return st;
    }
    auto enqueue = [&](int *n) -> int {
        const int e = enqueue_fixed(c, p, S.coeff, iters, S.kernel, T, &S.plan, &tail, prof, do_deriv, zero, S.persist);
        *n = c->info.jacobi_launches;
        return e;
    };
    int n = 0;
    if (p.use_graph && !p.profile) {
        GraphKey key{p.mode, S.persist ? HSFLOW_KERNEL_PERSIST : S.kernel, iters, T, c->info.tile_w, c->info.tile_h, c->info.threads,
                     c->info.groups_per_thread, zero ? 0 : c->cur, p.use_previous * 2 + (do_deriv ? 1 : 0), S.coeff};
        if ((st = run_captured(c, key, enqueue, &n))) return st;
        c->info.jacobi_launches = n;
    } else {
        if (S.persist && (st = configure_persist(c, S.plan.s, EpsMode::None, c->info.deriv_fused != 0, S.coeff))) return st;
        if ((st = enqueue(&n))) return st;
    }
    c->coef_valid = true;
    c->coef_mode = HSFLOW_MODE_CV;
    c->info.iterations_done = iters;
    if (S.persist && async) c->persist_unchecked = true;
    if (!async) {
        HS_HIP(c, hipStreamSynchronize(c->stream));
        if (S.persist && persist_error(c)) {
            persist_failed(c);
            c->cur ^= 1;
            hsflow_params q = p;
            if (q.kernel == HSFLOW_KERNEL_PERSIST) q.kernel = HSFLOW_KERNEL_STRIP;
            q.reuse_derivatives = 0;
            return solve_impl(c, &q, false);
        }
        prof.collect();
        if (c->dStamps && (S.kernel == HSFLOW_KERNEL_STRIP || S.kernel == HSFLOW_KERNEL_FOLD)) dump_stamps(c, S.plan.s.tiles);
    }
    return HSFLOW_OK;
}

int first_eps_hit(const unsigned *w, int n, double epsilon, float *last)
{
    for (int s = 0; s < n; s++) {
        std::memcpy(last, &w[s], sizeof(float));
        if ((double)*last < epsilon) return s;
    }
    return -1;
}

float witness_threshold(double epsilon)
{
    float thr = epsilon > 0 ? (float)epsilon : 0.f;
    if ((double)thr < epsilon) thr = std::nextafterf(thr, INFINITY);
    if (thr < FLT_MIN) thr = thr > 0.f ? FLT_MIN : 0.f;
    return thr;
}

int witness_pass(hsflow_ctx *c, const hsflow_params &p, const SolveSetup &S, const JPlan &tailp, int stride, bool do_deriv,
                 Profiler &prof, bool async, int *launches, bool *rerun)
{
    const int iters = (int)S.budget, T = S.T, cur0 = c->cur;
    const JPlan &plan = S.plan;
    int st = HSFLOW_OK;
    c->epsThr = witness_threshold(p.epsilon);
    const bool persist = S.persist && async;
    const int n_launch = (iters + T - 1) / T;
    const JPlan &lastp = iters % T ? tailp : plan;
    const JPlan &firstp = n_launch == 1 ? lastp : plan;
    if (persist && ((st = persist_reserve(c)) || (st = persist_prepare_flags(c, plan.s.tiles)))) return st;
    const EpsMode last_mode = async ? EpsMode::Witness : EpsMode::WitnessLast;
    const EpsLayout words{n_launch - 1 + (async ? 1 : 2), stride, n_launch - 1, plan_eps_stride(S.kernel, plan),
                          plan_eps_stride(S.kernel, persist ? plan : lastp)};
    if ((st = eps_reserve(c, words.slots, stride))) return st;
    const bool fuse_deriv = do_deriv && !p.profile && strip_deriv_fusable(c, firstp);
    c->info.deriv_fused = fuse_deriv;
    auto enqueue = [&](int *n) -> int {
        if (p.use_previous && (st = save_start(c))) return st;
        c->epsStride = stride;
        if (do_deriv && !fuse_deriv) {
            prof.begin(0);
            HS_HIP(c, launch_deriv(c));
            prof.end();
        }
        const int zero_w = p.use_previous ? 0 : 1;
        if (zero_w) c->cur = 0;
        if (persist) {
            c->epsPtr = c->dEpsTiles;
            prof.begin(1);
            const int e = enqueue_persist(c, plan.s, iters, EpsMode::Witness, fuse_deriv, zero_w, S.coeff);
            prof.end();
            if (e) return e;
        } else for (int L = 0; L < n_launch; L++) {
            const bool is_last = L == n_launch - 1;
            const int a = c->cur, b = a ^ 1;
            c->epsPtr = c->dEpsTiles + (size_t)L * stride;
            prof.begin(1);
            hipError_t e = launch_j(c, is_last ? lastp : plan, is_last ? last_mode : EpsMode::Witness, c->dU[a], c->dV[a], c->dU[b],
                                    c->dV[b], S.coeff, L == 0 ? zero_w : 0, L == 0 && fuse_deriv);
            prof.end();
            HS_HIP(c, e);
            c->cur = b;
        }
        *n = persist ? 1 : n_launch;
        if (async && !c->async_reduce) {
            c->epsPtr = c->dEps;
            c->epsStride = 1;
            return HSFLOW_OK;
        }
        return eps_collect_enqueue(c, words, async && c->hMark != nullptr);
    };
    if (p.use_graph && !p.profile) {
        GraphKey key{p.mode, persist ? HSFLOW_KERNEL_PERSIST : S.kernel, iters, T, c->info.tile_w, c->info.tile_h, c->info.threads,
                     c->info.groups_per_thread, p.use_previous ? c->cur : 0,
                     p.use_previous * 2 + (do_deriv ? 1 : 0) + (async ? 4 : 0) + (async && c->async_reduce ? 8 : 0), S.coeff, c->epsThr};
        if ((st = run_captured(c, key, enqueue, launches))) return st;
        c->epsPtr = c->dEps;
        c->epsStride = 1;
    } else {
        if (persist && (st = configure_persist(c, plan.s, EpsMode::Witness, fuse_deriv, S.coeff))) return st;
        if ((st = enqueue(launches))) return st;
    }
    c->coef_valid = true;
    c->coef_mode = HSFLOW_MODE_CV;
    if (persist) c->persist_unchecked = true;
    c->info.iterations_done = iters;
    c->info.jacobi_launches = *launches;
    if (async) {
        const int zero_in = (n_launch == 1 && !p.use_previous && !persist) ? 1 : 0;
        c->lastl = hsflow_ctx::LastLaunch{true, lastp, zero_in, S.coeff, c->epsThr, persist};
        c->pend.active = true;
        c->pend.params = p;
        c->pend.iters = iters; c->pend.launches = *launches; c->pend.cur0 = cur0;
        c->pend.words = words;
        c->pend.reduced = c->async_reduce;
        c->pend.marked_by_reduce = c->async_reduce && c->hMark != nullptr;
        return HSFLOW_OK;
    }
    HS_HIP(c, hipStreamSynchronize(c->stream));
    float last = 0.f;
    if (witness_proven(c->hEps, words.slots, p.epsilon, &last, true)) {
        c->info.last_eps = last;
        prof.collect();
        return HSFLOW_OK;
    }
    *rerun = true;
    c->info.eps_rerun = 1;
    c->cur = cur0;
    return p.use_previous ? restore_start(c) : HSFLOW_OK;
}

int exact_pass(hsflow_ctx *c, const hsflow_params &p, const SolveSetup &S, int stride, Profiler &prof, int launches)
{
    const int iters = (int)S.budget, T = S.T;
    int st = HSFLOW_OK, zero_in = p.use_previous ? 0 : 1, done = 0;
    if (zero_in) c->cur = 0;
    while (done < iters) {
        const int chunk = S.multi ? std::min(T, iters - done) : 1;
        JPlan cp = S.plan;
        if (S.multi && chunk != T && !make_jplan(c, S.kernel, chunk, p, cp))
            return fail(c, HSFLOW_E_SIZE, "no feasible launch plan for a chunk");
        const int a = c->cur, b = a ^ 1;
        c->epsPtr = c->dEpsTiles + (size_t)done * stride;
        prof.begin(1);
        hipError_t e = S.multi ? launch_j(c, cp, EpsMode::EverySweep, c->dU[a], c->dV[a], c->dU[b], c->dV[b], S.coeff, zero_in)
                               : launch_simple(c, true, c->dU[a], c->dV[a], c->dU[b], c->dV[b], S.coeff, zero_in);
        prof.end();
        HS_HIP(c, e);
        c->cur = b;
        zero_in = 0;
        done += chunk;
        launches++;
    }
    std::vector<unsigned> heps;
    if ((st = eps_collect(c, iters, heps))) return st;
    c->sweep_eps.resize((size_t)iters);
    std::memcpy(c->sweep_eps.data(), heps.data(), (size_t)iters * sizeof(float));
    float last = 0.f;
    const int hit = first_eps_hit(heps.data(), iters, p.epsilon, &last);
    if (hit >= 0 && hit + 1 < iters) {
        const int k = hit + 1;
        if (p.use_previous && (st = restore_start(c))) return st;
        JPlan kp, kt;
        int Tk = 1;
        if (S.multi) {
            Tk = std::min(T, k);
            if (!make_jplan(c, S.kernel, Tk, p, kp)) return fail(c, HSFLOW_E_SIZE, "no feasible launch plan for the re-run");
            if (k % Tk && !make_jplan(c, S.kernel, k % Tk, p, kt)) return fail(c, HSFLOW_E_SIZE, "no feasible launch plan for the re-run tail");
        }
        st = enqueue_fixed(c, p, S.coeff, k, S.kernel, Tk, &kp, &kt, prof, false, !p.use_previous);
        if (st) return st;
        launches += c->info.jacobi_launches;
        HS_HIP(c, hipStreamSynchronize(c->stream));
        c->info.iterations_done = k;
    } else {
        c->info.iterations_done = hit >= 0 ? hit + 1 : iters;
    }
    c->info.last_eps = last;
    c->info.jacobi_launches = launches;
    prof.collect();
    return HSFLOW_OK;
}

int solve_iter_eps(hsflow_ctx *c, const hsflow_params &p, const SolveSetup &S, Profiler &prof, bool async)
{
    const int iters = (int)S.budget, T = S.T, kernel = S.kernel;
    int st = HSFLOW_OK;
    bool witness = (kernel == HSFLOW_KERNEL_STRIP || kernel == HSFLOW_KERNEL_FOLD) && !c->force_exact && strip_has_witness(S.plan);
    const bool do_deriv = !(p.reuse_derivatives && c->coef_valid && c->coef_mode == HSFLOW_MODE_CV);
    if (p.use_previous) {
        const size_t px = (size_t)c->plane * c->N;
        if (!c->dUb) HS_HIP(c, hipMalloc((void **)&c->dUb, px * sizeof(float)));
        if (!c->dVb) HS_HIP(c, hipMalloc((void **)&c->dVb, px * sizeof(float)));
    }
    int stride = S.multi ? plan_eps_stride(kernel, S.plan) : 1;
    JPlan tailp;
    if (S.multi && iters % T) {
        if (!make_jplan(c, kernel, iters % T, p, tailp)) return fail(c, HSFLOW_E_SIZE, "no feasible launch plan for a chunk");
        if (witness && !strip_has_witness(tailp)) {
            JPlan alt;
            if (make_witness_jplan(c, kernel, iters % T, p, alt)) tailp = alt;
        }
        stride = std::max(stride, plan_eps_stride(kernel, tailp));
        if (witness && !S.persist && (async || iters % T > 1) && !strip_has_witness(tailp)) witness = false;
    }
    if (async && !witness)
        return fail(c, HSFLOW_E_ARG, "solve_async with ITER|EPS: this launch plan (core tile thinner than a strip) cannot run witness launches; "
                                     "use hsflow_solve or other tuning parameters");
    int launches = 0;
    if (witness) {
        bool rerun = false;
        if ((st = witness_pass(c, p, S, tailp, stride, do_deriv, prof, async, &launches, &rerun)) || !rerun) return st;
        if ((st = eps_prepare(c, iters, stride))) return st;
    } else {
        if (p.use_previous && (st = save_start(c))) return st;
        if ((st = eps_prepare(c, iters, stride))) return st;
        if (do_deriv) {
            prof.begin(0);
            HS_HIP(c, launch_deriv(c));
            prof.end();
        }
        c->coef_valid = true;
        c->coef_mode = HSFLOW_MODE_CV;
    }
    return exact_pass(c, p, S, stride, prof, launches);
}


int solve_eps_chunks(hsflow_ctx *c, const hsflow_params &p, const SolveSetup &S, Profiler &prof)
{
    const int kernel = S.kernel, T = S.T;
    const bool multi = S.multi;
    const long long budget = S.budget;
    int st = HSFLOW_OK;
    if (!p.use_previous) {
        c->cur = 0;
        HS_HIP(c, hipMemsetAsync(c->dU[0], 0, (size_t)c->plane * c->N * sizeof(float), c->stream));
        HS_HIP(c, hipMemsetAsync(c->dV[0], 0, (size_t)c->plane * c->N * sizeof(float), c->stream));
    }
    if (!(p.reuse_derivatives && c->coef_valid && c->coef_mode == HSFLOW_MODE_CV)) {
        prof.begin(0);
        HS_HIP(c, launch_deriv(c));
        prof.end();
    }
    c->coef_valid = true;
    c->coef_mode = HSFLOW_MODE_CV;
    long long done = 0;
    int launches = 0;
    float last = 0.f;
    bool stop = false;
    constexpr long long kStallSweeps = 4096, kMaxSweeps = 1LL << 24;
    float best_eps = INFINITY;
    long long best_at = 0;
    bool stalled = false;
    while (!stop) {
        const int chunk = (int)std::min<long long>(T, budget - done);
        JPlan cp = S.plan;
        if (multi && chunk != T && !make_jplan(c, kernel, chunk, p, cp))
            return fail(c, HSFLOW_E_SIZE, "no feasible launch plan for a chunk");
        const int a = c->cur, b = a ^ 1;
        const int n = multi ? chunk : 1;
        if ((st = eps_prepare(c, n, multi ? plan_eps_stride(kernel, cp) : 1))) return st;
        c->epsPtr = c->dEpsTiles;
        prof.begin(1);
        if (!multi)
            HS_HIP(c, launch_simple(c, true, c->dU[a], c->dV[a], c->dU[b], c->dV[b], S.coeff));
        else
            HS_HIP(c, launch_j(c, cp, EpsMode::EverySweep, c->dU[a], c->dV[a], c->dU[b], c->dV[b], S.coeff));
        prof.end();
        launches++;
        std::vector<unsigned> heps;
        if ((st = eps_collect(c, n, heps))) return st;
        const int hit = first_eps_hit(heps.data(), n, p.epsilon, &last);
        for (int s = 0; s < n && hit < 0; s++) {
            float e;
            std::memcpy(&e, &heps[(size_t)s], sizeof(float));
            if (e < best_eps) { best_eps = e; best_at = done + s; }
        }
        if (hit >= 0 && hit < n - 1) {
            JPlan rp;
            if (!make_jplan(c, kernel, hit + 1, p, rp))
                return fail(c, HSFLOW_E_SIZE, "no feasible launch plan for the replay");
            prof.begin(1);
            HS_HIP(c, launch_j(c, rp, EpsMode::None, c->dU[a], c->dV[a], c->dU[b], c->dV[b], S.coeff));
            prof.end();
            launches++;
            done += hit + 1;
            stop = true;
        } else {
            done += n;
            if (hit >= 0) stop = true;
        }
        c->cur = b;
        if (S.use_iter && p.max_iter > 0 && done >= budget) stop = true;
        if (!stop && budget > kMaxSweeps && (done - best_at >= kStallSweeps || done >= kMaxSweeps)) stop = stalled = true;
    }
    HS_HIP(c, hipStreamSynchronize(c->stream));
// ... 43 lines not shown
    if (use_eps && eps_windowed(c) && (kernel == HSFLOW_KERNEL_FOLD || kernel == HSFLOW_KERNEL_FUSED))
        return fail(c, HSFLOW_E_ARG, "EPS termination over a row window (hsflow_set_eps_rows) runs on the strip or the simple kernel");
    const bool multi = kernel != HSFLOW_KERNEL_SIMPLE;
    if (async && use_eps && !(use_iter && p.max_iter > 0 && p.max_iter <= (1 << 16) &&
                              (kernel == HSFLOW_KERNEL_STRIP || kernel == HSFLOW_KERNEL_FOLD) && !c->force_exact))
        return fail(c, HSFLOW_E_ARG, "solve_async with EPS termination needs ITER|EPS with a sweep budget and the strip / fold kernel "
                                     "(ITER-only termination works with every kernel)");
    const long long budget = (use_iter && p.max_iter > 0) ? p.max_iter : (1LL << 40);

    int T = 1;
    JPlan plan;
    hsflow_params eff = p;
    if (multi) {
        const int horizon = budget > (1 << 30) ? 64 : (int)budget;
        if (p.fuse_steps > 0) T = std::min(p.fuse_steps, kMaxFuse);
        else if (kernel == HSFLOW_KERNEL_STRIP || kernel == HSFLOW_KERNEL_FOLD)
            T = (use_eps && !(use_iter && p.max_iter > 0)) ? std::min(8, horizon)
                                                          : pick_strip_T(c, horizon, p, kernel == HSFLOW_KERNEL_FOLD);
        else T = pick_T(horizon, 0);
        if (budget < T) T = (int)budget;
        if ((kernel == HSFLOW_KERNEL_STRIP || kernel == HSFLOW_KERNEL_FOLD) && coeff < 1e-20f) T = std::min(T, 8);
        if (!make_jplan(c, kernel, T, p, plan))
            return fail(c, HSFLOW_E_SIZE, "no feasible launch plan for the requested tile/threads/rows/fuse_steps");
        if (use_eps && use_iter && p.max_iter > 0 && (kernel == HSFLOW_KERNEL_STRIP || kernel == HSFLOW_KERNEL_FOLD) &&
            !strip_has_witness(plan)) {
            JPlan alt;
            if (make_witness_jplan(c, kernel, T, p, alt)) plan = alt;
        }
        plan_to_info(c, plan);
    } else {
        c->info.fuse_steps = 1; c->info.tile_w = c->info.tile_h = 0; c->info.threads = 256;
        c->info.groups_per_thread = 1; c->info.tiles = 0; c->info.lds_bytes = 0;
    }
    c->info.kernel = kernel;
    bool persist = false;
    static const bool persist_auto = getenv("HSFLOW_PERSIST_AUTO") != nullptr;
    if (persist_asked || (persist_auto && p.kernel == HSFLOW_KERNEL_AUTO && kernel == HSFLOW_KERNEL_STRIP)) {
        const char *why = !(use_iter && p.max_iter > 0 && budget <= (1 << 16)) ? "needs a sweep budget (ITER)"
                                                                               : persist_obstacle(c, plan.s, (int)budget, p, async, use_eps);
        if (!why && use_eps && !strip_has_witness(plan)) why = "this launch plan cannot run witness phases";
        if (!why) persist = true;
        else if (persist_asked) return fail(c, HSFLOW_E_SIZE, std::string("HSFLOW_KERNEL_PERSIST: ") + why);
    }
    c->info.persistent = persist ? (int)((budget + T - 1) / T) : 0;
    S = SolveSetup{coeff, kernel, multi, use_iter, use_eps, budget, T, plan, persist, eff};
    return HSFLOW_OK;
}

int solve_impl_inner(hsflow_ctx *c, const hsflow_params *pp, bool async, bool *took_over);

int solve_impl(hsflow_ctx *c, const hsflow_params *pp, bool async)
{
    const hsflow_ctx::Pending owed = c ? c->pend : hsflow_ctx::Pending();
    bool took_over = false;
    const int st = solve_impl_inner(c, pp, async, &took_over);
    if (st && took_over && !c->pend.active) c->pend = owed;
    if (c) c->last_marked = false;
    if (!st && async && c->async_reduce && c->hMark) {
        const bool by_reduce = c->pend.active && c->pend.marked_by_reduce;
        if (!by_reduce) hipLaunchKernelGGL(hsk::k_mark_done, dim3(1), dim3(64), 0, c->stream, c->dSeq, c->hMarkDev);
        if (by_reduce || hipGetLastError() == hipSuccess) {
            c->mark_issued++;
            c->last_marked = true;
            c->flow_after_mark = false;
            if (c->pend.active) c->pend.mark = c->mark_issued;
        } else if (c->pend.active) c->pend.reduced = false;
    }
    return st;
}

int solve_impl_inner(hsflow_ctx *c, const hsflow_params *pp, bool async, bool *took_over)
{
    int st = check_ctx(c, 0);
    if (st) return st;
    const bool repeat = c->pend.active && async && !c->force_exact && pp && pp->struct_size == sizeof(hsflow_params) &&
                        !pp->use_previous && std::memcmp(pp, &c->pend.params, sizeof(hsflow_params)) == 0;
    if (repeat) { c->pend.active = false; *took_over = true; }
    else if ((st = settle_pending(c))) return st;
    c->lastl.valid = false;
    if (!pp || pp->struct_size != sizeof(hsflow_params))
        return fail(c, HSFLOW_E_ARG, "params null or struct_size mismatch");
    const hsflow_params &p = *pp;
    if (!c->frames_set) return fail(c, HSFLOW_E_STATE, "frames were not set");
    if (p.mode == HSFLOW_MODE_CLASSIC || p.mode == HSFLOW_MODE_CLASSIC_AS_SHIPPED) return solve_classic(c, p, async);
    if (p.mode != HSFLOW_MODE_CV) return fail(c, HSFLOW_E_ARG, "unknown mode");
    c->info.eps_rerun = 0;
    c->info.deriv_fused = 0;
    SolveSetup S;
    PlanKey key;
    std::memset(&key, 0, sizeof(key));
    key.p = p;
    key.p.use_previous = key.p.reuse_derivatives = key.p.use_graph = key.p.profile = 0;
    key.async = async ? 1 : 0;
    key.exact = c->force_exact ? 1 : 0;
    const bool cacheable = p.kernel != HSFLOW_KERNEL_PERSIST && !getenv("HSFLOW_PERSIST_AUTO");
    const PlanEntry *hit = nullptr;
    if (cacheable)
        for (const PlanEntry &e : c->plan_cache)
            if (std::memcmp(&e.key, &key, sizeof(key)) == 0) { hit = &e; break; }
    if (hit) {
        if ((st = check_solve_args(c, p, async))) return st;
        S = hit->S;
        S.eff = p;
        hsflow_info &i = c->info;
        const hsflow_info &j = hit->info;
        i.kernel = j.kernel; i.fuse_steps = j.fuse_steps; i.tile_w = j.tile_w; i.tile_h = j.tile_h; i.threads = j.threads;
        i.groups_per_thread = j.groups_per_thread; i.tiles = j.tiles; i.lds_bytes = j.lds_bytes; i.persistent = j.persistent;
    } else {
        if ((st = prepare_solve(c, p, async, S))) return st;
        if (cacheable) {
            if (c->plan_cache.size() >= 16) c->plan_cache.erase(c->plan_cache.begin());
            c->plan_cache.push_back(PlanEntry{key, S, c->info});
        }
    }
    c->info.deriv_ms = c->info.jacobi_ms = c->info.solve_ms = 0.f;
    c->info.last_eps = 0.f;
    Profiler prof{c, p.profile != 0};
    if (!S.use_eps) return solve_fixed(c, S.eff, S, prof, async);
    constexpr long long kSpecMax = 1 << 16;
    if (S.use_iter && p.max_iter > 0 && S.budget <= kSpecMax) return solve_iter_eps(c, S.eff, S, prof, async);
    return solve_eps_chunks(c, S.eff, S, prof);
}

int copy_frame_in(hsflow_ctx *c, uint8_t *dst, const void *src, size_t stride, hipMemcpyKind kind, bool sync)
{
    if (sync) HS_HIP(c, hipMemcpy2D(dst, c->P, src, stride, c->W, c->H, kind));
    else HS_HIP(c, hipMemcpy2DAsync(dst, c->P, src, stride, c->W, c->H, kind, c->stream));
    return HSFLOW_OK;
}

}
```

opticalflowhs_amd/csrc/hsflow.hip:

```cpp
#include "../../include/hsflow.h"
#include "hs_kernels.hip.h"
#include "hs_kernels_pre.hip.h"
#include "hs_kernels_classic.hip.h"
#include "hs_kernels_classic_strip.hip.h"
#include "hs_kernels_render.hip.h"
#include "hs_kernels_verify.hip.h"

#include <atomic>
#include <chrono>
#include <algorithm>
#include <cfloat>
#include <cmath>
#include <cstdio>
#include <cstdlib>
#include <cstring>
#include <map>
#include <mutex>
#include <string>
#include <tuple>
#include <type_traits>
#include <vector>

#include "hs_context.hip.h"
#include "hs_plan_launch.hip.h"
// ... 170 lines not shown
    }
    return HSFLOW_OK;
}

int hsflow_destroy(hsflow_ctx *c)
{
    if (!c) return HSFLOW_OK;
    hipSetDevice(c->device);
    if (c->stream || !c->own_stream) hipStreamSynchronize(c->stream);
    if (c->shadow) { hsflow_destroy(c->shadow); c->shadow = nullptr; }
    if (c->borrowed) c->dA = c->dB = nullptr;
    hipFree(c->dCmp);
    if (c->hCmp) hipHostFree(c->hCmp);
    if (c->evVerify) hipEventDestroy(c->evVerify);
    for (auto &kv : c->graphs) {
        if (kv.second.exec) hipGraphExecDestroy(kv.second.exec);
        if (kv.second.graph) hipGraphDestroy(kv.second.graph);
    }
    for (hipEvent_t e : c->events) hipEventDestroy(e);
    hipFree(c->dA); hipFree(c->dB); hipFree(c->dCoef);
    for (int i = 0; i < 3; i++) hipFree(c->dE[i]);
    for (int i = 0; i < 2; i++) { hipFree(c->dU[i]); hipFree(c->dV[i]); }
    hipFree(c->dEps);
    hipFree(c->dEpsTiles); hipFree(c->dUb); hipFree(c->dVb);
    hipFree(c->dUp); hipFree(c->dVp); hipFree(c->dFlags);
    hipFree(c->dSeq);
    hipFree(c->dZero);
    if (c->hMark) hipHostFree(c->hMark);
    if (c->hErr) hipHostFree(c->hErr);
    if (c->counted) g_live_ctx[c->device & 63]--;
    hipFree(c->dStamps);
    hipFree(c->dScratch);
    hipFree(c->dPrio); hipFree(c->dRgb);
    if (c->evRender) hipEventDestroy(c->evRender);
    if (c->hEps) hipHostFree(c->hEps);
    if (c->own_stream && c->stream) hipStreamDestroy(c->stream);
    delete c;
    return HSFLOW_OK;
}

int hsflow_set_frames_u8(hsflow_ctx *c, int pair, const uint8_t *prev, size_t ps, const uint8_t *curr, size_t cs)
{
    int st = check_ctx(c, pair);
    if (st) return st;
    if ((st = settle_pending(c))) return st;
    if (!prev || !curr) return fail(c, HSFLOW_E_ARG, "null frame pointer");
    if (ps < (size_t)c->W || cs < (size_t)c->W) return fail(c, HSFLOW_E_SIZE, "frame stride smaller than width");
    HS_HIP(c, hipStreamSynchronize(c->stream));
    if ((st = copy_frame_in(c, c->dA + pair * c->plane, prev, ps, hipMemcpyHostToDevice, true))) return st;
    if ((st = copy_frame_in(c, c->dB + pair * c->plane, curr, cs, hipMemcpyHostToDevice, true))) return st;
    c->frames_set = true;
    c->coef_valid = false;
    return HSFLOW_OK;
}

static hipError_t copy_rows_async(hsflow_ctx *c, void *dst, size_t dpitch, const void *src, size_t spitch, size_t rowb,
                                  size_t rows, hipMemcpyKind kind)
{
    if (dpitch == rowb && spitch == rowb) return hipMemcpyAsync(dst, src, rowb * rows, kind, c->stream);
    return hipMemcpy2DAsync(dst, dpitch, src, spitch, rowb, rows, kind, c->stream);
}

int hsflow_set_frames_u8_async(hsflow_ctx *c, int pair, const uint8_t *prev, size_t ps, const uint8_t *curr, size_t cs)
{
    int st = check_ctx(c, pair);
    if (st) return st;
    if ((st = settle_pending(c))) return st;
    if (!prev || !curr) return fail(c, HSFLOW_E_ARG, "null frame pointer");
    if (ps < (size_t)c->W || cs < (size_t)c->W) return fail(c, HSFLOW_E_SIZE, "frame stride smaller than width");
    HS_HIP(c, copy_rows_async(c, c->dA + pair * c->plane, c->P, prev, ps, c->W, c->H, hipMemcpyHostToDevice));
    HS_HIP(c, copy_rows_async(c, c->dB + pair * c->plane, c->P, curr, cs, c->W, c->H, hipMemcpyHostToDevice));
    c->frames_set = true;
    c->coef_valid = false;
    return HSFLOW_OK;
}

int hsflow_set_frames_u8_device(hsflow_ctx *c, int pair, const void *dprev, size_t ps, const void *dcurr, size_t cs)
{
    int st = check_ctx(c, pair);
    if (st) return st;
    if ((st = settle_pending(c))) return st;
    if (!dprev || !dcurr) return fail(c, HSFLOW_E_ARG, "null frame pointer");
    if (ps < (size_t)c->W || cs < (size_t)c->W) return fail(c, HSFLOW_E_SIZE, "frame stride smaller than width");
    {
        const dim3 grid((c->W + 1023) / 1024, (c->H + 3) / 4, 2), block(64, 4);
        const bool aligned = (((uintptr_t)dprev | (uintptr_t)dcurr | ps | cs) & 15u) == 0;
        uint8_t *dA = c->dA + pair * c->plane, *dB = c->dB + pair * c->plane;
        if (aligned)
            hipLaunchKernelGGL(hsk::k_copy_pair_u8<true>, grid, block, 0, c->stream, (const uint8_t *)dprev, (long long)ps, (const uint8_t *)dcurr,
                               (long long)cs, dA, dB, c->W, c->H, c->P);
        else
            hipLaunchKernelGGL(hsk::k_copy_pair_u8<false>, grid, block, 0, c->stream, (const uint8_t *)dprev, (long long)ps, (const uint8_t *)dcurr,
                               (long long)cs, dA, dB, c->W, c->H, c->P);
        HS_HIP(c, hipGetLastError());
    }
    c->frames_set = true;
    c->coef_valid = false;
    return HSFLOW_OK;
}

int hsflow_push_frame_u8(hsflow_ctx *c, int pair, const uint8_t *next, size_t ns)
{
    int st = check_ctx(c, pair);
    if (st) return st;
    if ((st = settle_pending(c))) return st;
    if (!next) return fail(c, HSFLOW_E_ARG, "null frame pointer");
    if (ns < (size_t)c->W) return fail(c, HSFLOW_E_SIZE, "frame stride smaller than width");
    if (!c->frames_set) return fail(c, HSFLOW_E_STATE, "push_frame needs a previous pair");
    HS_HIP(c, hipMemcpyAsync(c->dA + pair * c->plane, c->dB + pair * c->plane, (size_t)c->plane, hipMemcpyDeviceToDevice, c->stream));
    HS_HIP(c, hipStreamSynchronize(c->stream));
    if ((st = copy_frame_in(c, c->dB + pair * c->plane, next, ns, hipMemcpyHostToDevice, true))) return st;
    c->coef_valid = false;
    return HSFLOW_OK;
}

static int preprocess_frame(hsflow_ctx *c, uint8_t *dst, const uint8_t *host, size_t stride, bool colour, bool blur, int slot = 0,
                            bool sync = true)
{
    const size_t bgr_bytes = (size_t)c->W * 3 * c->H, gray_bytes = (size_t)c->plane;
    const size_t one = bgr_bytes + 2 * gray_bytes, need = 2 * one;
    if (c->scratch_bytes < need) {
        HS_HIP(c, hipStreamSynchronize(c->stream));
        hipFree(c->dScratch);
        c->dScratch = nullptr; c->scratch_bytes = 0;
        HS_HIP(c, hipMalloc(&c->dScratch, need));
        c->scratch_bytes = need;
    }
    uint8_t *dBgr = (uint8_t *)c->dScratch + (size_t)slot * one, *dGray = dBgr + bgr_bytes;
    const dim3 grid((c->W + 255) / 256, (c->H + 3) / 4), block(64, 4);
    if (sync) HS_HIP(c, hipStreamSynchronize(c->stream));
    if (colour) {
        if (sync) HS_HIP(c, hipMemcpy2D(dBgr, (size_t)c->W * 3, host, stride, (size_t)c->W * 3, c->H, hipMemcpyHostToDevice));
        else HS_HIP(c, copy_rows_async(c, dBgr, (size_t)c->W * 3, host, stride, (size_t)c->W * 3, c->H, hipMemcpyHostToDevice));
        hipLaunchKernelGGL(hsk::k_bgr2gray, grid, block, 0, c->stream, dBgr, (long long)c->W * 3, blur ? dGray : dst, c->W, c->H, c->P);
    } else {
        if (sync) HS_HIP(c, hipMemcpy2D(blur ? dGray : dst, c->P, host, stride, c->W, c->H, hipMemcpyHostToDevice));
        else HS_HIP(c, copy_rows_async(c, blur ? dGray : dst, c->P, host, stride, c->W, c->H, hipMemcpyHostToDevice));
    }
    if (blur) hipLaunchKernelGGL(hsk::k_box_blur3, grid, block, 0, c->stream, dGray, dst, c->W, c->H, c->P);
    HS_HIP(c, hipGetLastError());
    if (sync) HS_HIP(c, hipStreamSynchronize(c->stream));
    return HSFLOW_OK;
}

int hsflow_set_frames_bgr8(hsflow_ctx *c, int pair, const uint8_t *prev, size_t ps, const uint8_t *curr, size_t cs, int blur3x3)
{
    int st = check_ctx(c, pair);
    if (st) return st;
    if ((st = settle_pending(c))) return st;
    if (!prev || !curr) return fail(c, HSFLOW_E_ARG, "null frame pointer");
    if (ps < (size_t)c->W * 3 || cs < (size_t)c->W * 3) return fail(c, HSFLOW_E_SIZE, "colour frame stride smaller than 3*width");
    if ((st = preprocess_frame(c, c->dA + pair * c->plane, prev, ps, true, blur3x3 != 0))) return st;
    if ((st = preprocess_frame(c, c->dB + pair * c->plane, curr, cs, true, blur3x3 != 0))) return st;
    c->frames_set = true;
    c->coef_valid = false;
    return HSFLOW_OK;
}

int hsflow_set_frames_gray8_blur(hsflow_ctx *c, int pair, const uint8_t *prev, size_t ps, const uint8_t *curr, size_t cs)
{
    int st = check_ctx(c, pair);
    if (st) return st;
    if ((st = settle_pending(c))) return st;
    if (!prev || !curr) return fail(c, HSFLOW_E_ARG, "null frame pointer");
    if (ps < (size_t)c->W || cs < (size_t)c->W) return fail(c, HSFLOW_E_SIZE, "frame stride smaller than width");
    if ((st = preprocess_frame(c, c->dA + pair * c->plane, prev, ps, false, true))) return st;
    if ((st = preprocess_frame(c, c->dB + pair * c->plane, curr, cs, false, true))) return st;
    c->frames_set = true;
    c->coef_valid = false;
    return HSFLOW_OK;
}

int hsflow_set_frames_bgr8_async(hsflow_ctx *c, int pair, const uint8_t *prev, size_t ps, const uint8_t *curr, size_t cs, int blur3x3)
{
    int st = check_ctx(c, pair);
    if (st) return st;
    if ((st = settle_pending(c))) return st;
    if (!prev || !curr) return fail(c, HSFLOW_E_ARG, "null frame pointer");
// ... 24 lines not shown
    int st = check_ctx(c, 0);
    if (st) return st;
    if ((st = settle_pending(c))) return st;
    if (on && !c->hMark) {
        HS_HIP(c, hipMalloc((void **)&c->dSeq, 2 * sizeof(unsigned)));
        HS_HIP(c, hipMemsetAsync(c->dSeq, 0, 2 * sizeof(unsigned), c->stream));
        HS_HIP(c, hipHostMalloc((void **)&c->hMark, 64, hipHostMallocMapped | hipHostMallocCoherent));
        HS_HIP(c, hipHostGetDevicePointer((void **)&c->hMarkDev, c->hMark, 0));
        *c->hMark = 0u;
        c->mark_issued = 0;
    }
    c->last_marked = false;
    c->async_reduce = on != 0;
    return HSFLOW_OK;
}

int hsflow_set_eps_rows(hsflow_ctx *c, int first_row, int rows)
{
    int st = check_ctx(c, 0);
    if (st) return st;
    if (rows > 0 && (first_row < 0 || first_row + rows > c->H)) return fail(c, HSFLOW_E_SIZE, "Eps row window outside the frame");
    if ((st = settle_pending(c))) return st;
    const int r0 = rows > 0 ? first_row : 0, n = rows > 0 ? rows : 0;
    if (r0 != c->eps_row0 || n != c->eps_rows) {
        drop_graphs(c);
        c->plan_cache.clear();
        c->lastl.valid = false;
        c->eps_row0 = r0;
        c->eps_rows = n;
    }
    return HSFLOW_OK;
}

static int note_solve(hsflow_ctx *c, const hsflow_params *p, int st)
{
    if (!c) return st;
    c->vstate = st ? 2 : 1;
    if (!st) {
        c->vparams = *p;
        c->v_org = c->org; c->v_eps_row0 = c->eps_row0; c->v_eps_rows = c->eps_rows;
    }
    return st;
}

int hsflow_solve_probe(hsflow_ctx *c, const hsflow_params *pp, float *sweep_eps)
{
    int st = check_ctx(c, 0);
    if (st) return st;
    if (!pp || pp->struct_size != sizeof(hsflow_params)) return fail(c, HSFLOW_E_ARG, "params null or struct_size mismatch");
    if (!sweep_eps) return fail(c, HSFLOW_E_ARG, "sweep_eps is null");
    if (pp->mode != HSFLOW_MODE_CV) return fail(c, HSFLOW_E_ARG, "hsflow_solve_probe: CV mode only");
    if (pp->max_iter <= 0 || pp->max_iter > (1 << 16)) return fail(c, HSFLOW_E_ARG, "hsflow_solve_probe: max_iter must be 1 .. 65536");
    hsflow_params q = *pp;
    q.term_type = HSFLOW_TERM_ITER | HSFLOW_TERM_EPS;
    q.epsilon = 0.0;
    q.profile = 0;
    if (q.kernel == HSFLOW_KERNEL_PERSIST) q.kernel = HSFLOW_KERNEL_STRIP;
    c->force_exact = true;
    st = solve_impl(c, &q, false);
    c->force_exact = false;
    {
        hsflow_params v = *pp;
        v.term_type = HSFLOW_TERM_ITER;
        note_solve(c, &v, st);
    }
    if (st) return st;
    if ((int)c->sweep_eps.size() != pp->max_iter) return fail(c, HSFLOW_E_STATE, "hsflow_solve_probe: the per-sweep pass did not run");
    std::memcpy(sweep_eps, c->sweep_eps.data(), (size_t)pp->max_iter * sizeof(float));
    return HSFLOW_OK;
}

int hsflow_take_verdict(hsflow_ctx *c, int *proven)
{
    int st = check_ctx(c, 0);
    if (st) return st;
    if (!proven) return fail(c, HSFLOW_E_ARG, "proven is null");
    if (!c->pend.active) return fail(c, HSFLOW_E_STATE, "no asynchronous ITER|EPS solve is waiting for its early-stop check");
    *proven = 0;
    return settle_pending(c, proven);
}

int hsflow_solve(hsflow_ctx *c, const hsflow_params *p) { return note_solve(c, p, solve_impl(c, p, false)); }
int hsflow_solve_async(hsflow_ctx *c, const hsflow_params *p) { return note_solve(c, p, solve_impl(c, p, true)); }

int hsflow_wait_solve(hsflow_ctx *c)
{
    int st = check_ctx(c, 0);
    if (st) return st;
    if ((st = settle_pending(c))) return st;
    if (c->last_marked) { if ((st = wait_marker(c, c->mark_issued))) return st; }
    else HS_HIP(c, hipStreamSynchronize(c->stream));
    return check_persist(c);
}

int hsflow_synchronize(hsflow_ctx *c)
{
    int st = check_ctx(c, 0);
    if (st) return st;
    if ((st = settle_pending(c))) return st;
    HS_HIP(c, hipStreamSynchronize(c->stream));
    return check_persist(c);
}

int hsflow_get_flow(hsflow_ctx *c, int pair, float *u, size_t us, float *v, size_t vs)
{
    int st = check_ctx(c, pair);
    if (st) return st;
    if (!u || !v) return fail(c, HSFLOW_E_ARG, "null flow pointer");
    const size_t rowb = (size_t)c->W * 4;
    if ((us & 3) || (vs & 3) || us < rowb || vs < rowb) return fail(c, HSFLOW_E_SIZE, "flow stride must be a multiple of 4 and >= 4*width");
    if ((st = settle_pending(c))) return st;
    HS_HIP(c, hipStreamSynchronize(c->stream));
    if ((st = check_persist(c))) return st;
    HS_HIP(c, hipMemcpy2D(u, us, c->dU[c->cur] + pair * c->plane, (size_t)c->P * 4, rowb, c->H, hipMemcpyDeviceToHost));
    HS_HIP(c, hipMemcpy2D(v, vs, c->dV[c->cur] + pair * c->plane, (size_t)c->P * 4, rowb, c->H, hipMemcpyDeviceToHost));
    return HSFLOW_OK;
}

int hsflow_get_flow_async(hsflow_ctx *c, int pair, float *u, size_t us, float *v, size_t vs)
{
    int st = check_ctx(c, pair);
    if (st) return st;
    if (!u || !v) return fail(c, HSFLOW_E_ARG, "null flow pointer");
    const size_t rowb = (size_t)c->W * 4;
    if ((us & 3) || (vs & 3) || us < rowb || vs < rowb) return fail(c, HSFLOW_E_SIZE, "flow stride must be a multiple of 4 and >= 4*width");
    HS_HIP(c, copy_rows_async(c, u, us, c->dU[c->cur] + pair * c->plane, (size_t)c->P * 4, rowb, c->H, hipMemcpyDeviceToHost));
    HS_HIP(c, copy_rows_async(c, v, vs, c->dV[c->cur] + pair * c->plane, (size_t)c->P * 4, rowb, c->H, hipMemcpyDeviceToHost));
    c->flow_after_mark = true;
    return HSFLOW_OK;
}

static int flow_rows_args(hsflow_ctx *c, int pair, int row0, int nrows, const void *du, size_t us, const void *dv, size_t vs)
{
    int st = check_ctx(c, pair);
    if (st) return st;
    if (!du || !dv) return fail(c, HSFLOW_E_ARG, "null flow pointer");
    if (row0 < 0 || nrows <= 0 || row0 + nrows > c->H) return fail(c, HSFLOW_E_SIZE, "row range outside the frame");
    const size_t rowb = (size_t)c->W * 4;
    if ((us & 3) || (vs & 3) || us < rowb || vs < rowb) return fail(c, HSFLOW_E_SIZE, "flow stride must be a multiple of 4 and >= 4*width");
    return HSFLOW_OK;
}

int hsflow_flow_view_device(hsflow_ctx *c, int pair, const float **du, const float **dv, size_t *stride_bytes)
{
    int st = check_ctx(c, pair);
    if (st) return st;
    if (!du || !dv || !stride_bytes) return fail(c, HSFLOW_E_ARG, "null out pointer");
    if ((st = settle_pending(c))) return st;
    if (c->last_marked && !c->flow_after_mark) { if ((st = wait_marker(c, c->mark_issued))) return st; }
    else {
        HS_HIP(c, hipStreamSynchronize(c->stream));
        c->flow_after_mark = false;
    }
    if ((st = check_persist(c))) return st;
    *du = c->dU[c->cur] + pair * c->plane;
    *dv = c->dV[c->cur] + pair * c->plane;
    *stride_bytes = (size_t)c->P * sizeof(float);
    return HSFLOW_OK;
}

int hsflow_get_flow_device(hsflow_ctx *c, int pair, int row0, int nrows, void *du, size_t us, void *dv, size_t vs)
{
    int st = flow_rows_args(c, pair, row0, nrows, du, us, dv, vs);
    if (st) return st;
    if ((st = settle_pending(c))) return st;
    const size_t rowb = (size_t)c->W * 4;
// ... 157 lines not shown
```

opticalflowhs_amd/csrc/pair_pipeline.cpp:

```cpp
#include "../../include/hsflow.h"

#include <hip/hip_runtime.h>

#include <cstdlib>
#include <new>
#include <string>
#include <vector>

struct hsflow_pipeline {
    struct Slot {
        hsflow_ctx *ctx = nullptr;
        bool busy = false;
        uint64_t ticket = 0;
        float *u = nullptr, *v = nullptr;
        size_t us = 0, vs = 0;
        hsflow_info done;
        bool has_done = false;
        uint64_t done_ticket = 0;
        hipStream_t stream = nullptr;
        hipEvent_t ev = nullptr;
    };
    std::vector<Slot> slots;
    std::vector<hipStream_t> lanes;
    int device = 0;
// ... 100 lines not shown
            g_pipeline_create_error = std::string("hsflow_create: ") + hsflow_last_error(nullptr);
            hsflow_pipeline_destroy(pl);
            return st;
        }
        hsflow_set_async_reduce(s.ctx, 1);
        if (const char *ov = getenv("HSFLOW_PIPELINE_CU_SHARE")) {
            const int share = atoi(ov);
            if (share > 0) hsflow_set_cu_share(s.ctx, share);
        }
    }
    *out = pl;
    return HSFLOW_OK;
}

int hsflow_pipeline_destroy(hsflow_pipeline *pl)
{
    if (!pl) return HSFLOW_OK;
    if (!pl->lanes.empty()) hipSetDevice(pl->device);
    for (auto &s : pl->slots) {
        hsflow_destroy(s.ctx);
        if (s.ev) hipEventDestroy(s.ev);
    }
    for (hipStream_t l : pl->lanes) hipStreamDestroy(l);
    delete pl;
    return HSFLOW_OK;
}

int hsflow_pipeline_submit(hsflow_pipeline *pl, const uint8_t *prev, size_t ps, const uint8_t *curr, size_t cs,
                           float *u, size_t us, float *v, size_t vs, const hsflow_params *params, uint64_t *ticket)
{
    return hsflow_pipeline_submit_ex(pl, HSFLOW_FRAMES_GRAY8, prev, ps, curr, cs, u, us, v, vs, params, ticket);
}

int hsflow_pipeline_submit_ex(hsflow_pipeline *pl, int format, const uint8_t *prev, size_t ps, const uint8_t *curr, size_t cs,
                              float *u, size_t us, float *v, size_t vs, const hsflow_params *params, uint64_t *ticket)
{
    if (!pl) return HSFLOW_E_ARG;
    if (format < HSFLOW_FRAMES_GRAY8 || format > HSFLOW_FRAMES_BGR8_BLUR) return pfail(pl, HSFLOW_E_ARG, "unknown frame format");
    if (!params) return pfail(pl, HSFLOW_E_ARG, "params is null");
    if (!u || !v) return pfail(pl, HSFLOW_E_ARG, "null flow pointer");
    hsflow_pipeline::Slot &s = pl->slots[pl->next % pl->slots.size()];
    int st = finish_slot(pl, s);
    if (st) return st;
    switch (format) {
    case HSFLOW_FRAMES_GRAY8: st = hsflow_set_frames_u8_async(s.ctx, 0, prev, ps, curr, cs); break;
    case HSFLOW_FRAMES_GRAY8_BLUR: st = hsflow_set_frames_gray8_blur_async(s.ctx, 0, prev, ps, curr, cs); break;
    default: st = hsflow_set_frames_bgr8_async(s.ctx, 0, prev, ps, curr, cs, format == HSFLOW_FRAMES_BGR8_BLUR); break;
    }
    if (st) {
        hsflow_synchronize(s.ctx);
        return ctx_fail(pl, s.ctx, st, "upload of the frames");
    }
    hsflow_params shaped;
    const hsflow_params *use = params;
    if (params->struct_size == sizeof(hsflow_params)) { shaped = stream_shape(pl, *params); use = &shaped; }
    if ((st = hsflow_solve_async(s.ctx, use))) {
        hsflow_synchronize(s.ctx);
        return ctx_fail(pl, s.ctx, st, "hsflow_solve_async");
    }
    if ((st = hsflow_get_flow_async(s.ctx, 0, u, us, v, vs))) {
        hsflow_synchronize(s.ctx);
        return ctx_fail(pl, s.ctx, st, "hsflow_get_flow_async");
    }
    if (pl->lanes.size() != pl->slots.size() && hipEventRecord(s.ev, s.stream) != hipSuccess) {
        hsflow_synchronize(s.ctx);
        return pfail(pl, HSFLOW_E_DEVICE, "hipEventRecord failed");
    }
    s.busy = true;
    s.ticket = pl->next;
    s.u = u; s.v = v; s.us = us; s.vs = vs;
    if (ticket) *ticket = pl->next;
    pl->next++;
    return HSFLOW_OK;
}

int hsflow_pipeline_submit_device(hsflow_pipeline *pl, const void *d_prev, size_t ps, const void *d_curr, size_t cs,
                                  const hsflow_params *params, uint64_t *ticket)
{
    if (!pl) return HSFLOW_E_ARG;
    if (!params) return pfail(pl, HSFLOW_E_ARG, "params is null");
    hsflow_pipeline::Slot &s = pl->slots[pl->next % pl->slots.size()];
    int st = finish_slot(pl, s);
    if (st) return st;
    if ((st = hsflow_set_frames_u8_device(s.ctx, 0, d_prev, ps, d_curr, cs))) {
        hsflow_synchronize(s.ctx);
        return ctx_fail(pl, s.ctx, st, "hsflow_set_frames_u8_device");
    }
    hsflow_params shaped;
    const hsflow_params *use = params;
    if (params->struct_size == sizeof(hsflow_params)) { shaped = stream_shape(pl, *params); use = &shaped; }
    if ((st = hsflow_solve_async(s.ctx, use))) {
        hsflow_synchronize(s.ctx);
        return ctx_fail(pl, s.ctx, st, "hsflow_solve_async");
    }
    s.busy = true;
    s.ticket = pl->next;
    s.u = s.v = nullptr; s.us = s.vs = 0;
    if (ticket) *ticket = pl->next;
    pl->next++;
    return HSFLOW_OK;
}

int hsflow_pipeline_flow_device(hsflow_pipeline *pl, uint64_t ticket, const float **du, const float **dv, size_t *stride_bytes)
{
    if (!pl) return HSFLOW_E_ARG;
    if (!du || !dv || !stride_bytes) return pfail(pl, HSFLOW_E_ARG, "null out pointer");
    int st = hsflow_pipeline_wait(pl, ticket);
    if (st) return st;
    hsflow_pipeline::Slot &s = pl->slots[ticket % pl->slots.size()];
    if (s.busy || !s.has_done || s.done_ticket != ticket) return pfail(pl, HSFLOW_E_STATE, "the slot of that ticket has been reused by a later pair");
    if ((st = hsflow_flow_view_device(s.ctx, 0, du, dv, stride_bytes))) return ctx_fail(pl, s.ctx, st, "hsflow_flow_view_device");
    return HSFLOW_OK;
}

static hsflow_pipeline::Slot *slot_of_finished(hsflow_pipeline *pl, uint64_t ticket, int *st)
{
    if ((*st = hsflow_pipeline_wait(pl, ticket))) return nullptr;
    hsflow_pipeline::Slot &s = pl->slots[ticket % pl->slots.size()];
    if (s.busy || !s.has_done || s.done_ticket != ticket) {
        *st = pfail(pl, HSFLOW_E_STATE, "the slot of that ticket has been reused by a later pair");
        return nullptr;
    }
    return &s;
}

int hsflow_pipeline_render(hsflow_pipeline *pl, uint64_t ticket, const hsflow_render_params *rp, uint8_t *rgb, size_t stride)
{
    if (!pl) return HSFLOW_E_ARG;
    int st = HSFLOW_OK;
    hsflow_pipeline::Slot *s = slot_of_finished(pl, ticket, &st);
    if (!s) return st;
    if ((st = hsflow_render_flow(s->ctx, 0, rp, rgb, stride))) return ctx_fail(pl, s->ctx, st, "hsflow_render_flow");
    return HSFLOW_OK;
}

int hsflow_pipeline_render_device(hsflow_pipeline *pl, uint64_t ticket, const hsflow_render_params *rp, void *d_rgb, size_t stride)
{
    if (!pl) return HSFLOW_E_ARG;
    int st = HSFLOW_OK;
    hsflow_pipeline::Slot *s = slot_of_finished(pl, ticket, &st);
    if (!s) return st;
    if ((st = hsflow_render_flow_device(s->ctx, 0, rp, d_rgb, stride))) return ctx_fail(pl, s->ctx, st, "hsflow_render_flow_device");
    if (hipSetDevice(pl->device) != hipSuccess || hipEventRecord(s->ev, s->stream) != hipSuccess || hipEventSynchronize(s->ev) != hipSuccess)
        return pfail(pl, HSFLOW_E_DEVICE, "waiting for the slot's render failed");
    return HSFLOW_OK;
}

int hsflow_pipeline_verify(hsflow_pipeline *pl, uint64_t ticket, hsflow_verify_report *report)
{
    if (!pl) return HSFLOW_E_ARG;
    if (!report || report->struct_size != sizeof(hsflow_verify_report)) return pfail(pl, HSFLOW_E_ARG, "report null or struct_size mismatch");
    int st = HSFLOW_OK;
    hsflow_pipeline::Slot *s = slot_of_finished(pl, ticket, &st);
    if (!s) return st;
    if ((st = hsflow_verify(s->ctx, 0, report))) return ctx_fail(pl, s->ctx, st, "hsflow_verify");
    return HSFLOW_OK;
}

int hsflow_pipeline_wait(hsflow_pipeline *pl, uint64_t ticket)
{
    if (!pl) return HSFLOW_E_ARG;
    if (ticket >= pl->next) return pfail(pl, HSFLOW_E_ARG, "ticket was never issued");
    hsflow_pipeline::Slot &s = pl->slots[ticket % pl->slots.size()];
    if (!s.busy || s.ticket != ticket) return HSFLOW_OK;
    return finish_slot(pl, s);
}

int hsflow_pipeline_info(hsflow_pipeline *pl, uint64_t ticket, hsflow_info *out)
{
    if (!pl) return HSFLOW_E_ARG;
    if (!out || out->struct_size != sizeof(hsflow_info)) return pfail(pl, HSFLOW_E_ARG, "info null or struct_size mismatch");
    int st = hsflow_pipeline_wait(pl, ticket);
    if (st) return st;
    hsflow_pipeline::Slot &s = pl->slots[ticket % pl->slots.size()];
    if (!s.has_done || s.done_ticket != ticket) return pfail(pl, HSFLOW_E_STATE, "the slot of that ticket has been reused by a later pair");
    if (!s.busy) {
        hsflow_info info;
        info.struct_size = sizeof(info);
        if ((st = hsflow_get_info_ex(s.ctx, &info, 1))) return ctx_fail(pl, s.ctx, st, "hsflow_get_info_ex");
        s.done.last_eps = info.last_eps;
    }
    *out = s.done;
    return HSFLOW_OK;
}

int hsflow_pipeline_drain(hsflow_pipeline *pl)
{
    if (!pl) return HSFLOW_E_ARG;
    int first = HSFLOW_OK;
    for (auto &s : pl->slots) {
        const int st = finish_slot(pl, s);
        if (st && !first) first = st;
    }
    return first;
}

int hsflow_pipeline_depth(hsflow_pipeline *pl) { return pl ? (int)pl->slots.size() : 0; }

const char *hsflow_pipeline_last_error(hsflow_pipeline *pl) { return pl ? pl->err.c_str() : g_pipeline_create_error.c_str(); }

}
```

opticalflowhs_amd/pipeline.py:

```python
import ctypes
import weakref

import numpy as np

from . import _lib
from ._lib import HsflowError, HsflowInfo, HsflowVerifyReport, TERM_ITER
from .solver import _is_device_tensor, _render_host, _render_target, make_params, make_render_params


def pinned_empty(shape, dtype):
    lib = _lib.load()
    dtype = np.dtype(dtype)
    n = int(np.prod(shape)) * dtype.itemsize
    p = ctypes.c_void_p()
    st = lib.hsflow_host_alloc(ctypes.byref(p), max(n, 1))
    if st:
        raise HsflowError(st, (lib.hsflow_last_error(None) or b"").decode())
    buf = (ctypes.c_ubyte * max(n, 1)).from_address(p.value)
    weakref.finalize(buf, lib.hsflow_host_free, ctypes.c_void_p(p.value))
    return np.frombuffer(buf, dtype=dtype, count=int(np.prod(shape))).reshape(shape)


class _DeviceView(object):

# ... 7 lines not shown
        self._lib = _lib.load()
        self._h = ctypes.c_void_p()
        self.width, self.height = int(width), int(height)
        st = self._lib.hsflow_pipeline_create_lanes(ctypes.byref(self._h), int(device), self.width, self.height, int(depth),
                                                    int(depth if lanes is None else lanes))
        if st:
            self._h = None
            raise HsflowError(st, (self._lib.hsflow_pipeline_last_error(None) or b"").decode())
        self.depth = self._lib.hsflow_pipeline_depth(self._h)
        self._held = {}

    def _check(self, st):
        if st:
            raise HsflowError(st, (self._lib.hsflow_pipeline_last_error(self._h) or b"").decode())

    def submit(self, prev, curr, u_out, v_out, params=None, frames="gray", **kw):
        fmt = {"gray": _lib.FRAMES_GRAY8, "gray_blur": _lib.FRAMES_GRAY8_BLUR, "bgr": _lib.FRAMES_BGR8, "bgr_blur": _lib.FRAMES_BGR8_BLUR}[frames]
        colour = fmt >= _lib.FRAMES_BGR8
        for a in (prev, curr):
            want = (self.height, self.width, 3) if colour else (self.height, self.width)
            if not isinstance(a, np.ndarray) or a.dtype != np.uint8 or a.shape != want or a.strides[-1] != 1 or (colour and a.strides[1] != 3):
                raise ValueError("frames must be u8 arrays of shape %r with packed pixels" % (want,))
        for a, dt in ((u_out, np.float32), (v_out, np.float32)):
            if not isinstance(a, np.ndarray) or a.dtype != dt or a.shape != (self.height, self.width) or a.strides[1] != a.itemsize:
                raise ValueError("pipeline buffers must be (height, width) arrays: u8 frames, fp32 flow, unit column stride")
        if not (u_out.flags.writeable and v_out.flags.writeable):
            raise ValueError("flow outputs must be writeable")
        if params is None:
            kw.setdefault("term_type", TERM_ITER)
            params = make_params(**kw)
        t = ctypes.c_uint64()
        self._check(self._lib.hsflow_pipeline_submit_ex(
            self._h, fmt, ctypes.c_void_p(prev.ctypes.data), prev.strides[0], ctypes.c_void_p(curr.ctypes.data), curr.strides[0],
            ctypes.c_void_p(u_out.ctypes.data), u_out.strides[0], ctypes.c_void_p(v_out.ctypes.data), v_out.strides[0],
            ctypes.byref(params), ctypes.byref(t)))
        self._held.pop(t.value - self.depth, None)
        self._held[t.value] = (prev, curr, u_out, v_out)
        return t.value

    def submit_device(self, prev, curr, params=None, **kw):
        for a in (prev, curr):
            if not (hasattr(a, "is_cuda") and a.is_cuda) or str(a.dtype) != "torch.uint8" or tuple(a.shape) != (self.height, self.width) or a.stride(1) != 1:
                raise ValueError("device frames must be CUDA uint8 tensors of shape (height, width) with unit column stride")
        if params is None:
            kw.setdefault("term_type", TERM_ITER)
            params = make_params(**kw)
        t = ctypes.c_uint64()
        self._check(self._lib.hsflow_pipeline_submit_device(self._h, ctypes.c_void_p(prev.data_ptr()), prev.stride(0), ctypes.c_void_p(curr.data_ptr()),
                                                            curr.stride(0), ctypes.byref(params), ctypes.byref(t)))
        self._held.pop(t.value - self.depth, None)
        self._held[t.value] = (prev, curr)
        return t.value

    def flow_device(self, ticket, copy=True):
        import torch
        pu, pv, sb = ctypes.c_void_p(), ctypes.c_void_p(), ctypes.c_size_t()
        self._check(self._lib.hsflow_pipeline_flow_device(self._h, int(ticket), ctypes.byref(pu), ctypes.byref(pv), ctypes.byref(sb)))
        self._held.pop(int(ticket), None)
        out = []
        for p in (pu, pv):
            view = torch.as_tensor(_DeviceView(p.value, (self.height, self.width), (sb.value, 4)), device="cuda")
            out.append(view.clone() if copy else view)
        return tuple(out)

    def render(self, ticket, route="cv", out=None, params=None, **kw):
        rp = params if params is not None else make_render_params(route, **kw)
        if _is_device_tensor(out):
            ptr, stride = _render_target(out, self.height, self.width)
            self._check(self._lib.hsflow_pipeline_render_device(self._h, int(ticket), ctypes.byref(rp), ptr, stride))
            self._held.pop(int(ticket), None)
            return out
        img = _render_host(out, self.height, self.width)
        self._check(self._lib.hsflow_pipeline_render(self._h, int(ticket), ctypes.byref(rp), ctypes.c_void_p(img.ctypes.data), img.strides[0]))
        self._held.pop(int(ticket), None)
        return img

    def verify(self, ticket):
        r = HsflowVerifyReport()
        r.struct_size = ctypes.sizeof(HsflowVerifyReport)
        self._check(self._lib.hsflow_pipeline_verify(self._h, int(ticket), ctypes.byref(r)))
        self._held.pop(int(ticket), None)
        return r

    def wait(self, ticket):
        self._check(self._lib.hsflow_pipeline_wait(self._h, int(ticket)))
        self._held.pop(int(ticket), None)

    def info(self, ticket):
        i = HsflowInfo()
        i.struct_size = ctypes.sizeof(HsflowInfo)
        self._check(self._lib.hsflow_pipeline_info(self._h, int(ticket), ctypes.byref(i)))
        self._held.pop(int(ticket), None)
        return {name: getattr(i, name) for name, _ in HsflowInfo._fields_}

    def drain(self):
        self._check(self._lib.hsflow_pipeline_drain(self._h))
        self._held.clear()

    def close(self):
        if self._h is not None:
            self._lib.hsflow_pipeline_destroy(self._h)
            self._h = None
            self._held.clear()

    def __enter__(self):
        return self

    def __exit__(self, *a):
        self.close()

    def __del__(self):
        try:
            self.close()
        except Exception:
            pass
```

Measured before the change: 1.663 million Mpix*iter/s.

## Read device frames in place in the fused derivative strip kernel, skipping the staging copy

The device-frame submit path no longer launches a separate copy kernel into the context's frame buffers. The first fused derivative+Jacobi strip launch now reads the caller's frames directly using their own strides, and writes the interior bytes back into the internal buffers as it goes, so later reads and frame queries still work. The first launch is issued outside the captured graph and the remaining launches are replayed from a separate graph key. This removes one full read/write pass over both frames and a kernel launch per pair, at the cost of the first launch running outside the graph and extra stores inside the fused kernel.

```diff
diff --git a/include/hsflow.h b/include/hsflow.h
--- a/include/hsflow.h
+++ b/include/hsflow.h
@@ -113,6 +113,9 @@
 
 int hsflow_solve(hsflow_ctx *ctx, const hsflow_params *params);
 int hsflow_solve_async(hsflow_ctx *ctx, const hsflow_params *params);
+int hsflow_solve_async_frames_device(hsflow_ctx *ctx, const void *d_prev, size_t prev_stride, const void *d_curr,
+                                     size_t curr_stride, const hsflow_params *params);
+int hsflow_frame_copies_elided(hsflow_ctx *ctx, uint64_t *count);
 int hsflow_synchronize(hsflow_ctx *ctx);
 
 
@@ -207,9 +210,12 @@
 int hsflow_pipeline_render(hsflow_pipeline *pl, uint64_t ticket, const hsflow_render_params *rp, uint8_t *rgb, size_t stride);
 int hsflow_pipeline_render_device(hsflow_pipeline *pl, uint64_t ticket, const hsflow_render_params *rp, void *d_rgb, size_t stride);
 int hsflow_pipeline_verify(hsflow_pipeline *pl, uint64_t ticket, hsflow_verify_report *report);
+int hsflow_pipeline_frames_u8(hsflow_pipeline *pl, uint64_t ticket, uint8_t *prev, size_t prev_stride, uint8_t *curr,
+                              size_t curr_stride);
 int hsflow_pipeline_info(hsflow_pipeline *pl, uint64_t ticket, hsflow_info *info);
 int hsflow_pipeline_drain(hsflow_pipeline *pl);
 int hsflow_pipeline_depth(hsflow_pipeline *pl);
+int hsflow_pipeline_copies_elided(hsflow_pipeline *pl, uint64_t *count);
 const char *hsflow_pipeline_last_error(hsflow_pipeline *pl);
 
 
diff --git a/opticalflowhs_amd/_lib.py b/opticalflowhs_amd/_lib.py
--- a/opticalflowhs_amd/_lib.py
+++ b/opticalflowhs_amd/_lib.py
@@ -86,6 +86,8 @@
     "hsflow_push_frame_u8": (_i, [_vp, _i, _vp, _sz]),
     "hsflow_solve": (_i, [_vp, _pp]),
     "hsflow_solve_async": (_i, [_vp, _pp]),
+    "hsflow_solve_async_frames_device": (_i, [_vp, _vp, _sz, _vp, _sz, _pp]),
+    "hsflow_frame_copies_elided": (_i, [_vp, ctypes.POINTER(ctypes.c_uint64)]),
     "hsflow_synchronize": (_i, [_vp]),
     "hsflow_wait_solve": (_i, [_vp]),
     "hsflow_get_flow": (_i, [_vp, _i, _vp, _sz, _vp, _sz]),
@@ -128,6 +130,8 @@
     "hsflow_pipeline_info": (_i, [_vp, ctypes.c_uint64, ctypes.POINTER(HsflowInfo)]),
     "hsflow_pipeline_drain": (_i, [_vp]),
     "hsflow_pipeline_depth": (_i, [_vp]),
+    "hsflow_pipeline_copies_elided": (_i, [_vp, ctypes.POINTER(ctypes.c_uint64)]),
+    "hsflow_pipeline_frames_u8": (_i, [_vp, ctypes.c_uint64, _vp, _sz, _vp, _sz]),
     "hsflow_pipeline_last_error": (ctypes.c_char_p, [_vp]),
     "hsflow_multi_create": (_i, [ctypes.POINTER(_vp), ctypes.POINTER(_i), _i, _i, _i, _i]),
     "hsflow_multi_destroy": (_i, [_vp]),
diff --git a/opticalflowhs_amd/csrc/hs_context.hip.h b/opticalflowhs_amd/csrc/hs_context.hip.h
--- a/opticalflowhs_amd/csrc/hs_context.hip.h
+++ b/opticalflowhs_amd/csrc/hs_context.hip.h
@@ -135,6 +135,12 @@
     hipEvent_t evVerify = nullptr;
     size_t scratch_bytes = 0;
     int cur = 0;
+    struct FrameRef {
+        bool active = false;
+        const uint8_t *A = nullptr, *B = nullptr;
+        long long PA = 0, PB = 0;
+    } lazy, src;
+    unsigned long long copies_elided = 0;
     bool frames_set = false;
     bool coef_valid = false;
     hsflow_info info;
diff --git a/opticalflowhs_amd/csrc/hs_kernels_strip.hip.h b/opticalflowhs_amd/csrc/hs_kernels_strip.hip.h
--- a/opticalflowhs_amd/csrc/hs_kernels_strip.hip.h
+++ b/opticalflowhs_amd/csrc/hs_kernels_strip.hip.h
@@ -153,11 +153,18 @@
 #endif
 }
 
-template <int R>
+struct FrameSrc {
+    int PA, PB;
+    uint8_t *keepA, *keepB;
+};
+
+template <int R, bool EXT = false>
 __device__ __forceinline__ void strip_derive(const uint8_t *__restrict__ fA, const uint8_t *__restrict__ fB,
                                              const StripGeom &g, long long base, int x0, int y0, int dir, bool xin,
-                                             uint4 (&lc)[R])
-{
+                                             uint4 (&lc)[R], const FrameSrc fs = FrameSrc{0, 0, nullptr, nullptr},
+                                             const unsigned keep = 0)
+{
+    const int PA = EXT ? fs.PA : g.P, PB = EXT ? fs.PB : g.P;
     const int mode = xin ? 0 : ((x0 < 0 || (g.W & 3) == 0) ? 1 : 2);
     int xg = x0, xb[4] = {0, 0, 0, 0};
     unsigned flipx = 0;
@@ -175,10 +182,10 @@
     uint32_t wa[R + 2], wbv[R];
 #pragma unroll
     for (int j = 0; j < R + 2; j++)
-        wa[j] = *(const uint32_t *)(fA + base + (long long)mirror_index(y0 + dir * (j - 1), g.H) * g.P + (mode == 2 ? 0 : xg));
+        wa[j] = *(const uint32_t *)(fA + base + (long long)mirror_index(y0 + dir * (j - 1), g.H) * PA + (mode == 2 ? 0 : xg));
 #pragma unroll
     for (int r = 0; r < R; r++)
-        wbv[r] = *(const uint32_t *)(fB + base + (long long)mirror_index(y0 + dir * r, g.H) * g.P + (mode == 2 ? 0 : xg));
+        wbv[r] = *(const uint32_t *)(fB + base + (long long)mirror_index(y0 + dir * r, g.H) * PB + (mode == 2 ? 0 : xg));
     if (mode == 1) {
 #pragma unroll
         for (int j = 0; j < R + 2; j++) wa[j] = __builtin_bswap32(wa[j]);
@@ -191,9 +198,21 @@
                 return (uint32_t)row[xb[0]] | ((uint32_t)row[xb[1]] << 8) | ((uint32_t)row[xb[2]] << 16) | ((uint32_t)row[xb[3]] << 24);
             };
 #pragma unroll
-            for (int j = 0; j < R + 2; j++) wa[j] = bytes(fA + base + (long long)mirror_index(y0 + dir * (j - 1), g.H) * g.P);
-#pragma unroll
-            for (int r = 0; r < R; r++) wbv[r] = bytes(fB + base + (long long)mirror_index(y0 + dir * r, g.H) * g.P);
+            for (int j = 0; j < R + 2; j++) wa[j] = bytes(fA + base + (long long)mirror_index(y0 + dir * (j - 1), g.H) * PA);
+#pragma unroll
+            for (int r = 0; r < R; r++) wbv[r] = bytes(fB + base + (long long)mirror_index(y0 + dir * r, g.H) * PB);
+        }
+    }
+    if constexpr (EXT) {
+        if (fs.keepA != nullptr) {
+#pragma unroll
+            for (int r = 0; r < R; r++) {
+                if ((keep >> r) & 1u) {
+                    const long long o = base + (long long)(y0 + dir * r) * g.P + x0;
+                    *(uint32_t *)(fs.keepA + o) = wa[r + 1];
+                    *(uint32_t *)(fs.keepB + o) = wbv[r];
+                }
+            }
         }
     }
     int a[R + 2][6];
@@ -234,7 +253,7 @@
                                                         unsigned long long *__restrict__ stamps,
                                                         const float eps_thr, const uint8_t *__restrict__ fA,
                                                         const uint8_t *__restrict__ fB, uint32_t *__restrict__ coef_w,
-                                                        const PersistArgs pa = PersistArgs())
+                                                        const FrameSrc fs, const PersistArgs pa = PersistArgs())
 {
     static_assert(!PERSIST || EPS == 0 || EPS == 2, "the persistent form runs plain or witness phases");
     extern __shared__ __attribute__((aligned(16))) float4 ex[];
@@ -349,7 +368,15 @@
         }
     }
     if constexpr (DERIV) {
-        strip_derive<R>(fA, fB, g, base, x0, rev ? y0 + R - 1 : y0, rev ? -1 : 1, xin, lc);
+        unsigned keep = 0;
+        if (fs.keepA != nullptr && (x0 >= 0) && (x0 < g.W) && (4 * lane >= g.HX) && (4 * lane < g.HX + g.CW)) {
+#pragma unroll
+            for (int r = 0; r < R; r++) {
+                const int j = w * R + img_row(r), y = y0 + img_row(r);
+                if (j >= g.T && j < g.T + g.CH && y >= 0 && y < g.H) keep |= 1u << r;
+            }
+        }
+        strip_derive<R, true>(fA, fB, g, base, x0, rev ? y0 + R - 1 : y0, rev ? -1 : 1, xin, lc, fs, keep);
 #pragma unroll
         for (int r = 0; r < R; r++) unpack_row(r);
     }
@@ -729,12 +756,12 @@
                                                         const float eps_thr)
 {
     strip_body<R, NTMAX, EPS, E0, false>(coef, u_in, v_in, u_out, v_out, g, ilambda, eps_out, eps_stride, stamps, eps_thr,
-                                     nullptr, nullptr, nullptr);
+                                     nullptr, nullptr, nullptr, FrameSrc{0, 0, nullptr, nullptr});
 }
 
 template <int R, int NTMAX, int EPS, int E0>
 __global__ __launch_bounds__(NTMAX) void k_jacobi_strip_deriv(const uint8_t *__restrict__ fA,
-                                                              const uint8_t *__restrict__ fB,
+                                                              const uint8_t *__restrict__ fB, const FrameSrc fs,
                                                               uint32_t *__restrict__ coef_w,
                                                               const float *__restrict__ u_in,
                                                               const float *__restrict__ v_in,
@@ -746,7 +773,7 @@
                                                               const float eps_thr)
 {
     strip_body<R, NTMAX, EPS, E0, true>(nullptr, u_in, v_in, u_out, v_out, g, ilambda, eps_out, eps_stride, stamps, eps_thr,
-                                    fA, fB, coef_w);
+                                    fA, fB, coef_w, fs);
 }
 
 template <int R, int NTMAX, int EPS, int E0, bool DERIV>
@@ -761,7 +788,7 @@
                                                                 const float eps_thr, const PersistArgs pa)
 {
     strip_body<R, NTMAX, EPS, E0, DERIV, true>(coef_rw, u_in, v_in, nullptr, nullptr, g, ilambda, eps_out, eps_stride, stamps, eps_thr,
-                                               fA, fB, coef_rw, pa);
+                                               fA, fB, coef_rw, FrameSrc{g.P, g.P, nullptr, nullptr}, pa);
 }
 
 __device__ __forceinline__ float lane_xor32(float x, bool lower)
diff --git a/opticalflowhs_amd/csrc/hs_plan_launch.hip.h b/opticalflowhs_amd/csrc/hs_plan_launch.hip.h
--- a/opticalflowhs_amd/csrc/hs_plan_launch.hip.h
+++ b/opticalflowhs_amd/csrc/hs_plan_launch.hip.h
@@ -340,7 +340,12 @@
     constexpr auto kern = strip_kernel<R, NTMAX, (int)EPS, FOLD, DERIV, E0>();
     if (p.g.zero_in) ui = vi = c->dZero;
     unsigned long long *stamps = p.tiles <= 65536 ? c->dStamps : nullptr;
-    if constexpr (DERIV)
+    if constexpr (DERIV && !FOLD) {
+        const bool ext = c->src.active;
+        const hsk::FrameSrc fs{ext ? (int)c->src.PA : c->P, ext ? (int)c->src.PB : c->P, ext ? c->dA : nullptr, ext ? c->dB : nullptr};
+        return launch_lds<kern>(c, p.tiles, p.g.NW * 64, p.lds_bytes, ext ? c->src.A : c->dA, ext ? c->src.B : c->dB, fs, c->dCoef, ui, vi, uo, vo,
+                                p.g, coeff, c->epsPtr, c->epsStride, stamps, c->epsThr);
+    } else if constexpr (DERIV)
         return launch_lds<kern>(c, p.tiles, p.g.NW * 64, p.lds_bytes, c->dA, c->dB, c->dCoef, ui, vi, uo, vo, p.g, coeff, c->epsPtr,
                                 c->epsStride, stamps, c->epsThr);
     else
diff --git a/opticalflowhs_amd/csrc/hs_runtime.hip.h b/opticalflowhs_amd/csrc/hs_runtime.hip.h
--- a/opticalflowhs_amd/csrc/hs_runtime.hip.h
+++ b/opticalflowhs_amd/csrc/hs_runtime.hip.h
@@ -24,6 +24,40 @@
     if (pair < 0 || pair >= c->N) return fail(c, HSFLOW_E_ARG, "pair index out of range");
     if (hipSetDevice(c->device) != hipSuccess) return fail(c, HSFLOW_E_DEVICE, "hipSetDevice failed");
     (void)hipGetLastError();
+    return HSFLOW_OK;
+}
+
+hipError_t launch_frame_copy(hsflow_ctx *c, int pair, const void *dprev, size_t ps, const void *dcurr, size_t cs)
+{
+    const dim3 grid((c->W + 1023) / 1024, (c->H + 3) / 4, 2), block(64, 4);
+    const bool aligned = (((uintptr_t)dprev | (uintptr_t)dcurr | ps | cs) & 15u) == 0;
+    uint8_t *dA = c->dA + pair * c->plane, *dB = c->dB + pair * c->plane;
+    if (aligned)
+        hipLaunchKernelGGL(hsk::k_copy_pair_u8<true>, grid, block, 0, c->stream, (const uint8_t *)dprev, (long long)ps, (const uint8_t *)dcurr,
+                           (long long)cs, dA, dB, c->W, c->H, c->P);
+    else
+        hipLaunchKernelGGL(hsk::k_copy_pair_u8<false>, grid, block, 0, c->stream, (const uint8_t *)dprev, (long long)ps, (const uint8_t *)dcurr,
+                           (long long)cs, dA, dB, c->W, c->H, c->P);
+    return hipGetLastError();
+}
+
+bool frames_readable_in_place(const hsflow_ctx *c, const void *dprev, size_t ps, const void *dcurr, size_t cs)
+{
+    static const bool keep = getenv("HSFLOW_KEEP_FRAME_COPY") && atoi(getenv("HSFLOW_KEEP_FRAME_COPY")) != 0;
+    return !keep && c->N == 1 && (((uintptr_t)dprev | (uintptr_t)dcurr | ps | cs) & 3u) == 0 && ps <= (size_t)INT32_MAX && cs <= (size_t)INT32_MAX;
+}
+
+int resolve_lazy_frames(hsflow_ctx *c, bool in_place)
+{
+    if (!c->lazy.active) return HSFLOW_OK;
+    c->lazy.active = false;
+    if (in_place) {
+        c->src = c->lazy;
+        c->src.active = true;
+        c->copies_elided++;
+        return HSFLOW_OK;
+    }
+    HS_HIP(c, launch_frame_copy(c, 0, c->lazy.A, (size_t)c->lazy.PA, c->lazy.B, (size_t)c->lazy.PB));
     return HSFLOW_OK;
 }
 
@@ -147,13 +181,14 @@
 }
 
 int enqueue_fixed(hsflow_ctx *c, const hsflow_params &p, float coeff, int iters, int kernel, int T,
-                  const JPlan *plan, const JPlan *tail_plan, Profiler &prof, bool do_deriv, bool zero_flow, bool persist = false)
+                  const JPlan *plan, const JPlan *tail_plan, Profiler &prof, bool do_deriv, bool zero_flow, bool persist = false,
+                  int part = 0)
 {
     int zero_in = zero_flow ? 1 : 0;
-    if (zero_flow) c->cur = 0;
+    if (zero_flow && part != 2) c->cur = 0;
     bool fuse = do_deriv && !p.profile && kernel != HSFLOW_KERNEL_SIMPLE &&
                 strip_deriv_fusable(c, iters >= T ? *plan : *tail_plan);
-    if (do_deriv && !fuse) {
+    if (do_deriv && !fuse && part != 2) {
         prof.begin(0);
         HS_HIP(c, launch_deriv(c));
         prof.end();
@@ -176,6 +211,13 @@
             left -= 1;
         } else {
             const JPlan *pl = (left >= T) ? plan : tail_plan;
+            if (part == 2 && launches == 0) {
+                fuse = false;
+                left -= pl->T;
+                zero_in = 0;
+                launches++;
+                continue;
+            }
             prof.begin(1);
             HS_HIP(c, launch_j(c, *pl, EpsMode::None, c->dU[a], c->dV[a], c->dU[b], c->dV[b], coeff, zero_in, fuse));
             prof.end();
@@ -185,6 +227,7 @@
         c->cur = b;
         zero_in = 0;
         launches++;
+        if (part == 1) break;
     }
     c->info.jacobi_launches = launches;
     return HSFLOW_OK;
diff --git a/opticalflowhs_amd/csrc/hs_solve.hip.h b/opticalflowhs_amd/csrc/hs_solve.hip.h
--- a/opticalflowhs_amd/csrc/hs_solve.hip.h
+++ b/opticalflowhs_amd/csrc/hs_solve.hip.h
@@ -305,20 +305,35 @@
     if (S.persist) {
         if ((st = persist_reserve(c)) || (st = persist_prepare_flags(c, S.plan.s.tiles))) return st;
     }
+    const bool in_place = c->lazy.active && c->info.deriv_fused && !S.persist && (iters >= T ? S.plan : tail).kind == HSFLOW_KERNEL_STRIP;
+    if ((st = resolve_lazy_frames(c, in_place))) return st;
+    int part = 0;
     auto enqueue = [&](int *n) -> int {
-        const int e = enqueue_fixed(c, p, S.coeff, iters, S.kernel, T, &S.plan, &tail, prof, do_deriv, zero, S.persist);
+        const int e = enqueue_fixed(c, p, S.coeff, iters, S.kernel, T, &S.plan, &tail, prof, do_deriv, zero, S.persist, part);
         *n = c->info.jacobi_launches;
         return e;
     };
     int n = 0;
-    if (p.use_graph && !p.profile) {
+    if (p.use_graph && !p.profile && in_place) {
+        GraphKey key{p.mode, S.kernel, iters, T, c->info.tile_w, c->info.tile_h, c->info.threads,
+                     c->info.groups_per_thread, zero ? 0 : c->cur, p.use_previous * 2 + (do_deriv ? 1 : 0) + 16, S.coeff};
+        part = 1;
+        st = enqueue(&n);
+        c->src.active = false;
+        if (st) return st;
+        part = 2;
+        if (iters > T && (st = run_captured(c, key, enqueue, &n))) return st;
+        c->info.jacobi_launches = n;
+    } else if (p.use_graph && !p.profile) {
         GraphKey key{p.mode, S.persist ? HSFLOW_KERNEL_PERSIST : S.kernel, iters, T, c->info.tile_w, c->info.tile_h, c->info.threads,
                      c->info.groups_per_thread, zero ? 0 : c->cur, p.use_previous * 2 + (do_deriv ? 1 : 0), S.coeff};
         if ((st = run_captured(c, key, enqueue, &n))) return st;
         c->info.jacobi_launches = n;
     } else {
         if (S.persist && (st = configure_persist(c, S.plan.s, EpsMode::None, c->info.deriv_fused != 0, S.coeff))) return st;
-        if ((st = enqueue(&n))) return st;
+        st = enqueue(&n);
+        c->src.active = false;
+        if (st) return st;
     }
     c->coef_valid = true;
     c->coef_mode = HSFLOW_MODE_CV;
@@ -375,23 +390,26 @@
     if ((st = eps_reserve(c, words.slots, stride))) return st;
     const bool fuse_deriv = do_deriv && !p.profile && strip_deriv_fusable(c, firstp);
     c->info.deriv_fused = fuse_deriv;
+    const bool in_place = c->lazy.active && fuse_deriv && !persist && firstp.kind == HSFLOW_KERNEL_STRIP;
+    if ((st = resolve_lazy_frames(c, in_place))) return st;
+    int part = 0;
     auto enqueue = [&](int *n) -> int {
-        if (p.use_previous && (st = save_start(c))) return st;
+        if (part != 2 && p.use_previous && (st = save_start(c))) return st;
         c->epsStride = stride;
-        if (do_deriv && !fuse_deriv) {
+        if (part != 2 && do_deriv && !fuse_deriv) {
             prof.begin(0);
             HS_HIP(c, launch_deriv(c));
             prof.end();
         }
         const int zero_w = p.use_previous ? 0 : 1;
-        if (zero_w) c->cur = 0;
+        if (zero_w && part != 2) c->cur = 0;
         if (persist) {
             c->epsPtr = c->dEpsTiles;
             prof.begin(1);
             const int e = enqueue_persist(c, plan.s, iters, EpsMode::Witness, fuse_deriv, zero_w, S.coeff);
             prof.end();
             if (e) return e;
-        } else for (int L = 0; L < n_launch; L++) {
+        } else for (int L = part == 2 ? 1 : 0; L < (part == 1 ? 1 : n_launch); L++) {
             const bool is_last = L == n_launch - 1;
             const int a = c->cur, b = a ^ 1;
             c->epsPtr = c->dEpsTiles + (size_t)L * stride;
@@ -403,6 +421,7 @@
             c->cur = b;
         }
         *n = persist ? 1 : n_launch;
+        if (part == 1) return HSFLOW_OK;
         if (async && !c->async_reduce) {
             c->epsPtr = c->dEps;
             c->epsStride = 1;
@@ -410,16 +429,26 @@
         }
         return eps_collect_enqueue(c, words, async && c->hMark != nullptr);
     };
-    if (p.use_graph && !p.profile) {
+    if (p.use_graph && !p.profile && !(in_place && n_launch == 1)) {
         GraphKey key{p.mode, persist ? HSFLOW_KERNEL_PERSIST : S.kernel, iters, T, c->info.tile_w, c->info.tile_h, c->info.threads,
                      c->info.groups_per_thread, p.use_previous ? c->cur : 0,
-                     p.use_previous * 2 + (do_deriv ? 1 : 0) + (async ? 4 : 0) + (async && c->async_reduce ? 8 : 0), S.coeff, c->epsThr};
+                     p.use_previous * 2 + (do_deriv ? 1 : 0) + (async ? 4 : 0) + (async && c->async_reduce ? 8 : 0) + (in_place ? 16 : 0),
+                     S.coeff, c->epsThr};
+        if (in_place) {
+            part = 1;
+            st = enqueue(launches);
+            c->src.active = false;
+            if (st) return st;
+            part = 2;
+        }
         if ((st = run_captured(c, key, enqueue, launches))) return st;
         c->epsPtr = c->dEps;
         c->epsStride = 1;
     } else {
         if (persist && (st = configure_persist(c, plan.s, EpsMode::Witness, fuse_deriv, S.coeff))) return st;
-        if ((st = enqueue(launches))) return st;
+        st = enqueue(launches);
+        c->src.active = false;
+        if (st) return st;
     }
     c->coef_valid = true;
     c->coef_mode = HSFLOW_MODE_CV;
@@ -533,6 +562,7 @@
         if ((st = witness_pass(c, p, S, tailp, stride, do_deriv, prof, async, &launches, &rerun)) || !rerun) return st;
         if ((st = eps_prepare(c, iters, stride))) return st;
     } else {
+        if ((st = resolve_lazy_frames(c, false))) return st;
         if (p.use_previous && (st = save_start(c))) return st;
         if ((st = eps_prepare(c, iters, stride))) return st;
         if (do_deriv) {
@@ -742,7 +772,10 @@
         return fail(c, HSFLOW_E_ARG, "params null or struct_size mismatch");
     const hsflow_params &p = *pp;
     if (!c->frames_set) return fail(c, HSFLOW_E_STATE, "frames were not set");
-    if (p.mode == HSFLOW_MODE_CLASSIC || p.mode == HSFLOW_MODE_CLASSIC_AS_SHIPPED) return solve_classic(c, p, async);
+    if (p.mode == HSFLOW_MODE_CLASSIC || p.mode == HSFLOW_MODE_CLASSIC_AS_SHIPPED) {
+        if ((st = resolve_lazy_frames(c, false))) return st;
+        return solve_classic(c, p, async);
+    }
     if (p.mode != HSFLOW_MODE_CV) return fail(c, HSFLOW_E_ARG, "unknown mode");
     c->info.eps_rerun = 0;
     c->info.deriv_fused = 0;
@@ -779,6 +812,7 @@
     if (!S.use_eps) return solve_fixed(c, S.eff, S, prof, async);
     constexpr long long kSpecMax = 1 << 16;
     if (S.use_iter && p.max_iter > 0 && S.budget <= kSpecMax) return solve_iter_eps(c, S.eff, S, prof, async);
+    if ((st = resolve_lazy_frames(c, false))) return st;
     return solve_eps_chunks(c, S.eff, S, prof);
 }
 
diff --git a/opticalflowhs_amd/csrc/hsflow.hip b/opticalflowhs_amd/csrc/hsflow.hip
--- a/opticalflowhs_amd/csrc/hsflow.hip
+++ b/opticalflowhs_amd/csrc/hsflow.hip
@@ -276,18 +276,7 @@
     if ((st = settle_pending(c))) return st;
     if (!dprev || !dcurr) return fail(c, HSFLOW_E_ARG, "null frame pointer");
     if (ps < (size_t)c->W || cs < (size_t)c->W) return fail(c, HSFLOW_E_SIZE, "frame stride smaller than width");
-    {
-        const dim3 grid((c->W + 1023) / 1024, (c->H + 3) / 4, 2), block(64, 4);
-        const bool aligned = (((uintptr_t)dprev | (uintptr_t)dcurr | ps | cs) & 15u) == 0;
-        uint8_t *dA = c->dA + pair * c->plane, *dB = c->dB + pair * c->plane;
-        if (aligned)
-            hipLaunchKernelGGL(hsk::k_copy_pair_u8<true>, grid, block, 0, c->stream, (const uint8_t *)dprev, (long long)ps, (const uint8_t *)dcurr,
-                               (long long)cs, dA, dB, c->W, c->H, c->P);
-        else
-            hipLaunchKernelGGL(hsk::k_copy_pair_u8<false>, grid, block, 0, c->stream, (const uint8_t *)dprev, (long long)ps, (const uint8_t *)dcurr,
-                               (long long)cs, dA, dB, c->W, c->H, c->P);
-        HS_HIP(c, hipGetLastError());
-    }
+    HS_HIP(c, launch_frame_copy(c, pair, dprev, ps, dcurr, cs));
     c->frames_set = true;
     c->coef_valid = false;
     return HSFLOW_OK;
@@ -478,6 +467,34 @@
 
 int hsflow_solve(hsflow_ctx *c, const hsflow_params *p) { return note_solve(c, p, solve_impl(c, p, false)); }
 int hsflow_solve_async(hsflow_ctx *c, const hsflow_params *p) { return note_solve(c, p, solve_impl(c, p, true)); }
+
+int hsflow_solve_async_frames_device(hsflow_ctx *c, const void *dprev, size_t ps, const void *dcurr, size_t cs, const hsflow_params *p)
+{
+    int st = check_ctx(c, 0);
+    if (st) return st;
+    if (!dprev || !dcurr || !frames_readable_in_place(c, dprev, ps, dcurr, cs)) {
+        if ((st = hsflow_set_frames_u8_device(c, 0, dprev, ps, dcurr, cs))) return st;
+        return hsflow_solve_async(c, p);
+    }
+    if ((st = settle_pending(c))) return st;
+    if (ps < (size_t)c->W || cs < (size_t)c->W) return fail(c, HSFLOW_E_SIZE, "frame stride smaller than width");
+    c->lazy.active = true;
+    c->lazy.A = (const uint8_t *)dprev; c->lazy.B = (const uint8_t *)dcurr;
+    c->lazy.PA = (long long)ps; c->lazy.PB = (long long)cs;
+    c->frames_set = true;
+    c->coef_valid = false;
+    st = note_solve(c, p, solve_impl(c, p, true));
+    c->src.active = false;
+    const int st2 = resolve_lazy_frames(c, false);
+    return st ? st : st2;
+}
+
+int hsflow_frame_copies_elided(hsflow_ctx *c, uint64_t *count)
+{
+    if (!c || !count) return HSFLOW_E_ARG;
+    *count = c->copies_elided;
+    return HSFLOW_OK;
+}
 
 int hsflow_wait_solve(hsflow_ctx *c)
 {
diff --git a/opticalflowhs_amd/csrc/pair_pipeline.cpp b/opticalflowhs_amd/csrc/pair_pipeline.cpp
--- a/opticalflowhs_amd/csrc/pair_pipeline.cpp
+++ b/opticalflowhs_amd/csrc/pair_pipeline.cpp
@@ -206,16 +206,12 @@
     hsflow_pipeline::Slot &s = pl->slots[pl->next % pl->slots.size()];
     int st = finish_slot(pl, s);
     if (st) return st;
-    if ((st = hsflow_set_frames_u8_device(s.ctx, 0, d_prev, ps, d_curr, cs))) {
-        hsflow_synchronize(s.ctx);
-        return ctx_fail(pl, s.ctx, st, "hsflow_set_frames_u8_device");
-    }
     hsflow_params shaped;
     const hsflow_params *use = params;
     if (params->struct_size == sizeof(hsflow_params)) { shaped = stream_shape(pl, *params); use = &shaped; }
-    if ((st = hsflow_solve_async(s.ctx, use))) {
-        hsflow_synchronize(s.ctx);
-        return ctx_fail(pl, s.ctx, st, "hsflow_solve_async");
+    if ((st = hsflow_solve_async_frames_device(s.ctx, d_prev, ps, d_curr, cs, use))) {
+        hsflow_synchronize(s.ctx);
+        return ctx_fail(pl, s.ctx, st, "hsflow_solve_async_frames_device");
     }
     s.busy = true;
     s.ticket = pl->next;
@@ -278,6 +274,16 @@
     hsflow_pipeline::Slot *s = slot_of_finished(pl, ticket, &st);
     if (!s) return st;
     if ((st = hsflow_verify(s->ctx, 0, report))) return ctx_fail(pl, s->ctx, st, "hsflow_verify");
+    return HSFLOW_OK;
+}
+
+int hsflow_pipeline_frames_u8(hsflow_pipeline *pl, uint64_t ticket, uint8_t *prev, size_t ps, uint8_t *curr, size_t cs)
+{
+    if (!pl) return HSFLOW_E_ARG;
+    int st = HSFLOW_OK;
+    hsflow_pipeline::Slot *s = slot_of_finished(pl, ticket, &st);
+    if (!s) return st;
+    if ((st = hsflow_get_frames_u8(s->ctx, 0, prev, ps, curr, cs))) return ctx_fail(pl, s->ctx, st, "hsflow_get_frames_u8");
     return HSFLOW_OK;
 }
 
@@ -319,6 +325,19 @@
     return first;
 }
 
+int hsflow_pipeline_copies_elided(hsflow_pipeline *pl, uint64_t *count)
+{
+    if (!pl || !count) return HSFLOW_E_ARG;
+    *count = 0;
+    for (auto &s : pl->slots) {
+        uint64_t n = 0;
+        const int st = hsflow_frame_copies_elided(s.ctx, &n);
+        if (st) return st;
+        *count += n;
+    }
+    return HSFLOW_OK;
+}
+
 int hsflow_pipeline_depth(hsflow_pipeline *pl) { return pl ? (int)pl->slots.size() : 0; }
 
 const char *hsflow_pipeline_last_error(hsflow_pipeline *pl) { return pl ? pl->err.c_str() : g_pipeline_create_error.c_str(); }
diff --git a/opticalflowhs_amd/pipeline.py b/opticalflowhs_amd/pipeline.py
--- a/opticalflowhs_amd/pipeline.py
+++ b/opticalflowhs_amd/pipeline.py
@@ -113,6 +113,19 @@
         self._held.pop(int(ticket), None)
         return r
 
+    def frames(self, ticket):
+        a = np.empty((self.height, self.width), np.uint8)
+        b = np.empty((self.height, self.width), np.uint8)
+        self._check(self._lib.hsflow_pipeline_frames_u8(self._h, int(ticket), ctypes.c_void_p(a.ctypes.data), a.strides[0],
+                                                        ctypes.c_void_p(b.ctypes.data), b.strides[0]))
+        self._held.pop(int(ticket), None)
+        return a, b
+
+    def copies_elided(self):
+        n = ctypes.c_uint64()
+        self._check(self._lib.hsflow_pipeline_copies_elided(self._h, ctypes.byref(n)))
+        return n.value
+
     def wait(self, ticket):
         self._check(self._lib.hsflow_pipeline_wait(self._h, int(ticket)))
         self._held.pop(int(ticket), None)
```

Result: faster. 1.708 million Mpix*iter/s, median of 6 (+2.7%).
